# jonaselgammal/GPry

Hardware: AMD Instinct MI355X
Metric: gp_refit_plus_nora_acq_cycle_throughput (higher is better)
Workload: dtype f64

## Files before the change

gpry_amd/_lib.py:

```python
import ctypes as C
import ctypes as _ct
import os

import numpy as np

_HERE = os.path.dirname(os.path.abspath(__file__))
LIB_PATH = os.path.join(_HERE, "libgpry_hip.so")

GPRY_MAX_DIM = 32
MASK_CLASSIFIED_INF = 1
MASK_OUTSIDE_TRUST = 2

KERNEL_IDS = {"rbf": 0, "matern12": 1, "matern32": 2, "matern52": 3}
KERNEL_WHITE = 0x10


class GpryAffine(C.Structure):
    _fields_ = [("has_x_affine", C.c_int),
                ("x_lo", C.c_double * GPRY_MAX_DIM),
                ("x_span", C.c_double * GPRY_MAX_DIM),
                ("y_mean", C.c_double), ("y_std", C.c_double),
                ("clip_hi", C.c_double)]


# ... 40 lines not shown
    "gpry_ns_generation_clustered": (C.c_int, [_vp, _vp, _vp, _vp, _vp, C.c_int64, C.c_double, _vp, C.c_uint64,
                                               C.c_int64, C.c_int, C.c_int, _vp, C.c_int, _vp, _vp, _vp,
                                               _P(C.c_double)]),
    "gpry_ns_generation_volumes": (C.c_int, [_vp, _vp, _vp, _vp, _vp, C.c_int64, C.c_double, _vp, C.c_uint64,
                                             C.c_int64, C.c_int, C.c_int, _vp, C.c_int, _vp, _vp, _vp, _vp,
                                             _P(C.c_double)]),
    "gpry_ns_generation_phantoms": (C.c_int, [_vp, _vp, _vp, _vp, _vp, C.c_int64, C.c_double, _vp, C.c_uint64,
                                              C.c_int64, C.c_int, C.c_int, _vp, C.c_int, _vp, _vp, _vp, _vp, C.c_int,
                                              _vp, _vp, _P(C.c_double)]),
    "gpry_ns_knn": (C.c_int, [_vp, _vp, _vp, _vp, C.c_int64, C.c_int, _vp, _P(C.c_double)]),
    "gpry_mcmc_chains": (C.c_int, [_vp, _vp, _vp, _vp, _vp, C.c_int64, _vp, C.c_double, C.c_double, C.c_uint64,
                                   C.c_int64, C.c_int, C.c_int, _vp, _vp, _vp, _vp, _vp, _vp, _vp, _vp, _P(C.c_double)]),
    "gpry_mcmc_ladders": (C.c_int, [_vp, _vp, _vp, _vp, _vp, C.c_int64, C.c_int, _vp, _vp, C.c_double, C.c_uint64,
                                    C.c_int64, C.c_int, C.c_int, C.c_int] + [_vp] * 11 + [_P(C.c_double)]),
    "gpry_hmc_chains": (C.c_int, [_vp, _vp, _vp, _vp, _vp, C.c_int64, _vp, C.c_double, C.c_int, C.c_double, C.c_double,
                                  C.c_uint64, C.c_int64, C.c_int, C.c_int] + [_vp] * 12),
    "gpry_hmc_chains_reflect": (C.c_int, [_vp, _vp, _vp, _vp, _vp, C.c_int64, _vp, C.c_double, C.c_int, C.c_double,
                                          C.c_double, C.c_uint64, C.c_int64, C.c_int, C.c_int] + [_vp] * 11
                                + [C.c_int, C.c_int, _vp, _vp]),
    "gpry_maximize_mean": (C.c_int, [_vp, _vp, _vp, _vp, _vp, C.c_int64, _vp, _vp, C.c_int, C.c_int, C.c_double,
                                     C.c_double, C.c_double] + [_vp] * 12 + [_P(C.c_double)]),
    "gpry_maximize_acq": (C.c_int, [_vp, _vp, _vp, _vp, C.c_int64, _vp, _vp, C.c_double, C.c_double, C.c_double, C.c_int,
                                    C.c_int, C.c_double, C.c_double, C.c_double] + [_vp] * 14 + [_P(C.c_double)]),
    "gpry_hessian_mean": (C.c_int, [_vp, _vp, C.c_int64, _vp, _vp, _vp, _P(C.c_double)]),
    "gpry_mean_theta_grad": (C.c_int, [_vp, _vp, C.c_int64, _vp, _vp, _P(C.c_double)]),
    "gpry_predict_thetas": (C.c_int, [_vp, _vp, C.c_int64, _vp, C.c_int64, _vp, _vp, _vp, _P(C.c_double)]),
    "gpry_predict_thetas_var": (C.c_int, [_vp, _vp, C.c_int64, _vp, C.c_int64, _vp, _vp, _vp, _vp, _P(C.c_double)]),
    "gpry_predict_cov": (C.c_int, [_vp, _vp, C.c_int64, _vp, _vp, _vp, _P(C.c_double)]),
    "gpry_sample_joint": (C.c_int, [_vp, _vp, C.c_int64, _vp, C.c_int64, C.c_uint64, C.c_double, _vp, _vp, _vp, _vp,
                                    _P(C.c_int), _P(C.c_double), _P(C.c_double)]),
    "gpry_loo": (C.c_int, [_vp, _vp, _vp, _vp, _vp, _vp, _P(C.c_double)]),
    "gpry_svm_fit": (C.c_int, [_vp, _vp, _vp, C.c_int64, C.c_int64, C.c_double, C.c_double, C.c_double, C.c_int64, _vp,
                               _P(C.c_double), _P(C.c_double), _P(C.c_double), _P(C.c_int64), _P(C.c_int), _P(C.c_double)]),
    "gpry_leave_out": (C.c_int, [_vp, _vp, _vp, C.c_int64, _vp, _vp, _vp, _vp, _vp, _P(C.c_double)]),
    "gpry_predict_without": (C.c_int, [_vp, _vp, _vp, C.c_int64, _vp, C.c_int64, _vp, _vp, _vp, _P(C.c_double)]),
    "gpry_var_theta_grad": (C.c_int, [_vp, _vp, C.c_int64, _vp, _vp, _P(C.c_double)]),
    "gpry_var_theta_grad_panel": (C.c_int64, [_vp]),
    "gpry_predict_grad": (C.c_int, [_vp, _vp, C.c_int, _vp, _vp, _vp]),
    "gpry_predict_grad_batch": (C.c_int, [_vp, _vp, C.c_int64, C.c_int, _vp, _vp, _vp, _vp]),
    "gpry_predict_point": (C.c_int, [_vp, _vp, C.c_int, C.c_int, _vp, _vp, _vp, _vp, _vp]),
    "gpry_set_gates": (C.c_int, [_vp, _vp, _vp, C.c_int64, C.c_double, C.c_double, C.c_int, _vp]),
    "gpry_sweep_logexp": (C.c_int, [_vp, _vp, C.c_int64, _vp, C.c_double, C.c_double,
                                    C.c_double, _vp, _vp, _vp, _P(C.c_int64)]),
    "gpry_sweep_logexp_given": (C.c_int, [_vp, _vp, C.c_int64, _vp, _vp, _vp, C.c_double, C.c_double,
                                          C.c_double, _vp, _vp, _vp, _P(C.c_int64)]),
    "gpry_sweep_fetch": (C.c_int, [_vp, C.c_int64, _vp, _vp, _vp]),
    "gpry_sweep_prune_info": (C.c_int, [_vp, _vp, _vp]),
    "gpry_sweep_screen_info": (C.c_int, [_vp, _vp]),
    "gpry_sweep_topk": (C.c_int, [_vp, C.c_int64, _vp, C.c_int64, _vp, _P(C.c_int64),
                                  _P(C.c_double)]),
    "gpry_kb_reset": (C.c_int, [_vp]),
    "gpry_kb_register": (C.c_int, [_vp, _vp, C.c_int64, _P(C.c_int64), _vp]),
    "gpry_kb_gram": (C.c_int, [_vp, C.c_int64, _vp, _vp, _P(C.c_int64)]),
    "gpry_kb_gram_rows": (C.c_int, [_vp, _vp, C.c_int64, _vp, _vp, _P(C.c_int64)]),
    "gpry_kb_rank": (C.c_int, [_vp, _vp, C.c_int64, _vp, C.c_int64, _vp, _vp, _vp, _vp, C.c_int64, _vp, C.c_int64, _vp,
                               C.c_int64, _vp, _vp, _vp, _vp, _vp, _P(C.c_int64), _P(C.c_int64), _vp]),
    "gpry_comm_unique_id": (C.c_int, [_vp]),
    "gpry_comm_init": (C.c_int, [_vp, C.c_int, C.c_int, _vp, _P(_vp)]),
    "gpry_comm_destroy": (C.c_int, [_vp]),
    "gpry_comm_info": (C.c_int, [_vp, _P(C.c_int), _P(C.c_int), _P(C.c_int)]),
    "gpry_comm_allgather": (C.c_int, [_vp, _vp, C.c_int64, _vp]),
    "gpry_comm_allreduce_max": (C.c_int, [_vp, _vp, C.c_int64]),
    "gpry_comm_barrier": (C.c_int, [_vp]),
    "gpry_group_create": (C.c_int, [C.c_int, _P(C.c_int), _vp, _P(_vp)]),
    "gpry_group_destroy": (C.c_int, [_vp]),
    "gpry_group_size": (C.c_int, [_vp, _P(C.c_int), _P(C.c_int)]),
    "gpry_group_member": (_vp, [_vp, C.c_int]),
    "gpry_group_last_error": (C.c_char_p, [_vp]),
    "gpry_group_set_model": (C.c_int, [_vp, _vp, _vp, _vp, C.c_int64, C.c_int, C.c_int, _vp,
                                       _P(GpryAffine), _P(C.c_int)]),
    "gpry_group_set_gates": (C.c_int, [_vp, _vp, _vp, C.c_int64, C.c_double, C.c_double, C.c_int, _vp]),
    "gpry_group_sweep_logexp": (C.c_int, [_vp, _vp, C.c_int64, _vp, C.c_double, C.c_double,
                                          C.c_double, _vp, _vp, _vp, _P(C.c_int64)]),
    "gpry_group_sweep_logexp_given": (C.c_int, [_vp, _vp, C.c_int64, _vp, _vp, _vp, C.c_double, C.c_double,
                                                C.c_double, _vp, _vp, _vp, _P(C.c_int64)]),
    "gpry_group_sweep_fetch": (C.c_int, [_vp, C.c_int64, _vp, _vp, _vp]),
    "gpry_group_sweep_topk": (C.c_int, [_vp, C.c_int64, _vp, C.c_int64, _vp, _P(C.c_int64),
                                        _P(C.c_double), _P(C.c_int)]),
    "gpry_group_lml_batch": (C.c_int, [_vp, _vp, C.c_int, C.c_int, _vp, _vp, _vp]),
    "gpry_timing_reset": (C.c_int, [_vp]),
    "gpry_timing_get": (C.c_int, [_vp, C.c_char_p, _P(C.c_double), _P(C.c_int64)]),
    "gpry_sweep_info": (C.c_int, [_vp, _P(C.c_int), _vp]),
    "gpry_microbench": (C.c_int, [_vp, C.c_int, C.c_int64, _P(C.c_double)]),
    "gpry_debug_gemm": (C.c_int, [_vp, _vp, _vp, _vp] + [C.c_int] * 9),
    "gpry_debug_logexp": (C.c_int, [_vp, _vp, _vp, C.c_int64, C.c_double, C.c_double, C.c_double, _vp]),
}


def _given_arrays(y_given, sigma_given, M):
    if y_given is None:
        raise ValueError("sigma_given without y_given")
    y_given = np.ascontiguousarray(y_given, dtype=np.float64)
    if y_given.shape != (M,):
        raise ValueError(f"y_given has shape {y_given.shape}, the pool has {M} rows")
    if sigma_given is not None:
        sigma_given = np.ascontiguousarray(sigma_given, dtype=np.float64)
        if sigma_given.shape != (M,):
            raise ValueError(f"sigma_given has shape {sigma_given.shape}, the pool has {M} rows")
    return y_given, sigma_given


MAX_STATUS = ("CONVERGED_G", "CONVERGED_F", "STALLED", "MAXITER", "BAD_START", "BAD_GRADIENT")


class GpryHipError(RuntimeError):
    """An API / HIP / RCCL failure reported by libgpry_hip.so."""


_lib = None


def load_library(path=None):
    global _lib
    if _lib is not None and path is None:
        return _lib
    p = path or os.environ.get("GPRY_HIP_LIB", LIB_PATH)
    if not os.path.exists(p):
        raise GpryHipError(
            f"{p} not found. Build it with `python -c 'import __graft_entry__ as g; "
            "g.build()'` or `make -C gpry_amd/csrc`. There is no CPU fallback.")
    lib = C.CDLL(p)
    for name, (res, args) in SIGNATURES.items():
        fn = getattr(lib, name)
        fn.restype, fn.argtypes = res, args
    _lib = lib
    return lib


def _ptr(a):
    return None if a is None else a.ctypes.data_as(C.c_void_p)


def _ptrs(arrays, *keys):
    return [_ptr(arrays.get(k)) for k in keys]


_CHAIN_OUT = ("X", "y", "X_last", "y_last", "naccept", "ncalls")
_BFGS_OUT = ("iters", "ncalls", "ngrad", "status")
_BFGS_TR = ("G_tr", "nhalv_tr", "reset_tr")


def _f64(a, shape=None):
    a = np.ascontiguousarray(a, dtype=np.float64)
    if shape is not None and a.shape != shape:
        raise ValueError(f"expected shape {shape}, got {a.shape}")
    return a


def device_count():
    n = C.c_int(0)
    lib = load_library()
    if lib.gpry_device_count(C.byref(n)) != 0:
        return 0
    return n.value


def make_affine(x_lo=None, x_span=None, y_mean=0.0, y_std=1.0, clip_hi=np.inf):
    tf = GpryAffine()
    tf.has_x_affine = 0 if x_lo is None else 1
    if x_lo is not None:
        for k in range(len(x_lo)):
            tf.x_lo[k] = float(x_lo[k])
            tf.x_span[k] = float(x_span[k])
    tf.y_mean, tf.y_std = float(y_mean), float(y_std)
    tf.clip_hi = float(clip_hi)
    return tf
# ... 689 lines not shown
    def sweep_topk(self, Kp, exclude=None):
        Kp = int(Kp)
        top = np.zeros(max(Kp, 1), dtype=CAND_DTYPE)
        n_out, bound = C.c_int64(0), C.c_double(0.0)
        if exclude is not None and len(exclude):
            exclude = np.ascontiguousarray(np.sort(np.asarray(exclude, dtype=np.int64)))
            nex = len(exclude)
        else:
            exclude, nex = None, 0
        self._check(self._lib.gpry_sweep_topk(self._h, Kp, _ptr(exclude), nex, _ptr(top),
                                              C.byref(n_out), C.byref(bound)), "gpry_sweep_topk")
        return top[:n_out.value], bound.value

    def kb_reset(self):
        self._check(self._lib.gpry_kb_reset(self._h), "gpry_kb_reset")

    def kb_register(self, X, want_var0=True):
        X = _f64(X)
        m = X.shape[0]
        first = C.c_int64(0)
        var0 = np.empty(m) if want_var0 else None
        self._check(self._lib.gpry_kb_register(self._h, _ptr(X), m, C.byref(first), _ptr(var0)),
                    "gpry_kb_register")
        return first.value, var0

    def kb_gram(self, p, n):
        G, kv = np.empty(n), np.empty(n)
        nn = C.c_int64(0)
        self._check(self._lib.gpry_kb_gram(self._h, int(p), _ptr(G), _ptr(kv), C.byref(nn)),
                    "gpry_kb_gram")
        if nn.value != n:
            raise GpryHipError(f"kb_gram: device holds {nn.value} candidates, host expected {n}")
        return G, kv

    def kb_gram_rows(self, p, n):
        p = np.ascontiguousarray(p, dtype=np.int64)
        G, kv = np.empty((len(p), n)), np.empty((len(p), n))
        nn = C.c_int64(0)
        self._check(self._lib.gpry_kb_gram_rows(self._h, _ptr(p), len(p), _ptr(G), _ptr(kv), C.byref(nn)),
                    "gpry_kb_gram_rows")
        if nn.value != n:
            raise GpryHipError(f"kb_gram_rows: device holds {nn.value} candidates, host expected {n}")
        return G, kv

    def kb_rank(self, X_new, var0, idx, y, sigma, acq, order, params, slots):
        m_new = 0 if X_new is None else len(X_new)
        X_new = None if m_new == 0 else _f64(X_new)
        params = _f64(params)
        counter, info = C.c_int64(0), C.c_int64(0)
        stats = np.zeros(3, dtype=np.int64)
        s_idx, s_y, s_sigma, s_acq, s_cond = slots
        for a, t in ((var0, np.float64), (idx, np.int64), (y, np.float64), (sigma, np.float64), (acq, np.float64),
                     (order, np.int64), (s_idx, np.int64), (s_y, np.float64), (s_sigma, np.float64),
                     (s_acq, np.float64), (s_cond, np.float64)):
            if a.dtype != t or not a.flags.c_contiguous:
                raise ValueError("kb_rank: arrays must be contiguous int64 / float64")
        if not (len(y) == len(sigma) == len(acq) == len(idx)) or len(params) != 5 or \
                not (len(s_idx) == len(s_y) == len(s_sigma) == len(s_acq) == len(s_cond)):
            raise ValueError("kb_rank: array lengths do not match")
        self._check(self._lib.gpry_kb_rank(self._h, _ptr(X_new), m_new, _ptr(var0), len(var0), _ptr(idx), _ptr(y),
                                           _ptr(sigma), _ptr(acq), len(idx), _ptr(order), len(order), _ptr(params),
                                           len(s_idx) - 1, _ptr(s_idx), _ptr(s_y), _ptr(s_sigma), _ptr(s_acq),
                                           _ptr(s_cond), C.byref(counter), C.byref(info), _ptr(stats)), "gpry_kb_rank")
        return counter.value, info.value, stats

    def timing_reset(self):
        self._check(self._lib.gpry_timing_reset(self._h), "gpry_timing_reset")

    def timing(self, name):
        ms, cnt = C.c_double(0.0), C.c_int64(0)
        self._lib.gpry_timing_get(self._h, name.encode(), C.byref(ms), C.byref(cnt))
        return ms.value, cnt.value

    def debug_gemm(self, A, B, C0, M, N, K, a_trans=False, b_trans=False, epi=0, kmode=0,
                   lower_only=False, tile_map=0):
        A, B = _f64(A), _f64(B)
        crow = (M + 127) // 128 if epi == 3 else M
        Cout = np.ascontiguousarray(np.zeros((crow, N)) if C0 is None else C0, dtype=np.float64).copy()
        self._check(self._lib.gpry_debug_gemm(self._h, _ptr(A), _ptr(B), _ptr(Cout), M, N, K,
                                              int(a_trans), int(b_trans), int(epi), int(kmode),
                                              int(lower_only), int(tile_map)), "gpry_debug_gemm")
        return Cout

    def debug_logexp(self, mu, sigma, zeta, baseline, sigma_n):
        mu, sigma = _f64(mu), _f64(sigma)
        acq = np.empty(len(mu))
        self._check(self._lib.gpry_debug_logexp(self._h, _ptr(mu), _ptr(sigma), len(mu), float(zeta),
                                                float(baseline), float(sigma_n), _ptr(acq)), "gpry_debug_logexp")
        return acq


    def microbench(self, kind, nbytes=0):
        v = C.c_double(0.0)
        self._check(self._lib.gpry_microbench(self._h, int(kind), int(nbytes), C.byref(v)),
                    "gpry_microbench")
        return v.value


class DeviceGroup:

    def __init__(self, devices, adopt=None):
        self._lib = load_library()
        devices = [int(v) for v in devices]
        if not devices:
            raise ValueError("DeviceGroup needs at least one device")
        self.devices = devices
        self._adopt = adopt
        arr = (C.c_int * len(devices))(*devices)
        self._h = C.c_void_p()
        rc = self._lib.gpry_group_create(len(devices), arr, adopt._h if adopt is not None else None,
                                         C.byref(self._h))
        if rc != 0:
            msg = self._lib.gpry_group_last_error(None).decode(errors="replace")
            self._h = None
            raise GpryHipError(f"gpry_group_create({devices}) failed ({rc}): {msg}")
        n, tr = C.c_int(0), C.c_int(0)
        self._lib.gpry_group_size(self._h, C.byref(n), C.byref(tr))
        self.size, self.transport = n.value, {0: "host", 1: "rccl"}[tr.value]
        self.note = self._lib.gpry_group_last_error(self._h).decode(errors="replace")
        self.sweep_epoch = 0
        self._sweep_M = 0
        self.d = 0

    def _check(self, rc, what):
        if rc != 0:
            msg = self._lib.gpry_group_last_error(self._h).decode(errors="replace")
            raise GpryHipError(f"{what} failed ({rc}): {msg}")

    def close(self):
        if getattr(self, "_h", None):
            try:
                self._lib.gpry_group_destroy(self._h)
            except Exception:
                pass
            self._h = None

    def __del__(self):
        self.close()

    def member(self, i):
        h = self._lib.gpry_group_member(self._h, int(i))
        if not h:
            raise IndexError(i)
        v = Device._view(h, self.devices[i])
        v._group = self
        return v

    def set_model(self, X_, y_, alpha, kernel_id, theta, affine=None):
        X_ = _f64(X_)
        N, d = X_.shape
        y_ = _f64(y_, (N,))
        alpha = _f64(np.broadcast_to(alpha, (N,)))
        if int(kernel_id) & KERNEL_WHITE:
            raise NotImplementedError("a device group does not carry the white term (WhiteKernel) of the kernel yet")
        theta = _f64(theta, (d + 1,))
        tf = make_affine(*affine) if affine is not None else None
        info = C.c_int(0)
        self._check(self._lib.gpry_group_set_model(self._h, _ptr(X_), _ptr(y_), _ptr(alpha), N, d, int(kernel_id),
                                                   _ptr(theta), C.byref(tf) if tf is not None else None,
                                                   C.byref(info)), "gpry_group_set_model")
        self.d = d
        return info.value

    def set_gates(self, sv=None, coef=None, gamma=0.0, intercept=0.0, positive_is_finite=True,
                  trust_bounds=None):
        n_sv = 0
# ... 113 lines not shown
```

gpry_amd/csrc/api.hip:

```cpp
#include "sweep.h"
#include "kb_gram.h"
#include <algorithm>

int require_model(gpry_ctx* ctx, bool need_factor) {
    if (ctx->N <= 0) return gpry_fail(ctx, -1, "no training set (call gpry_set_train)");
    if (!ctx->have_theta) return gpry_fail(ctx, -1, "no hyperparameters (call gpry_set_theta)");
    if (need_factor && !ctx->factor_valid) return gpry_fail(ctx, -1, "model not factorised (call gpry_factorize)");
    if (need_factor && ctx->tf.has_x_affine)
        for (int k = 0; k < ctx->d; k++)
            if (!(ctx->tf.x_span[k] != 0.0) || !isfinite(ctx->tf.x_span[k]) || !isfinite(ctx->tf.x_lo[k]))
                return gpry_fail(ctx, -1, "affine map of X: span %g, offset %g in dimension %d of %d (gpry_set_affine of another model?)",
                                 ctx->tf.x_span[k], ctx->tf.x_lo[k], k, ctx->d);
    return 0;
}


static int copy_out_matrix(gpry_ctx* ctx, const double* dsrc, int64_t ld, int64_t rows, int64_t cols, double* hdst) {
    HIP_TRY(ctx, hipMemcpy2DAsync(hdst, sizeof(double) * cols, dsrc, sizeof(double) * ld,
                                  sizeof(double) * cols, rows, hipMemcpyDeviceToHost, ctx->stream));
    HIP_TRY(ctx, hipStreamSynchronize(ctx->stream));
    return 0;
}

bool panel_timed_out(int marker) { return (marker & 0xFF00) == 0x5A00; }
int panel_timeout_error(gpry_ctx* ctx, int marker) {
    return gpry_fail(ctx, -2, "Cholesky panel step timed out (wait %d; the GPU is shared with work that starves the step?)", marker & 0xFF);
}

int objective_entry(gpry_ctx* ctx, const char* name, const double* thetas, int64_t B) {
    GPRY_TRY(serve_stop(ctx));
    if (ctx->N <= 0) return gpry_fail(ctx, -1, "%s: no training set (call gpry_set_train)", name);
    const int w = ctx_ntheta(ctx);
    for (int64_t i = 0; i < B * w; i++)
        if (!isfinite(thetas[i]))
            return gpry_fail(ctx, -1, "%s: theta[%d] of evaluation %lld is not finite", name, (int)(i % w), (long long)(i / w));
    if (ctx->d > 32) return gpry_fail(ctx, -1, "%s: d > 32 is not supported", name);
    HIP_TRY(ctx, hipSetDevice(ctx->device));
    ctx->lml_cache = false;
    return 0;
}
int objective_row(gpry_ctx* ctx, int64_t bytes, int info_at, double** hres, double** dres) {
    GPRY_TRY(ensure_pinned(ctx, bytes));
    *hres = static_cast<double*>(ctx->hpin);
    *dres = static_cast<double*>(ctx->hpin_dev);
    objective_row_unwritten(*hres, info_at);
    return 0;
}
int objective_status(gpry_ctx* ctx, const char* name, int64_t which, const double* row, int info_at, int* info) {
    if (row[info_at] < 0.0) return gpry_fail(ctx, -2, "%s: evaluation %lld did not deliver its status", name, (long long)which);
    if (panel_timed_out((int)row[info_at + 2])) return panel_timeout_error(ctx, (int)row[info_at + 2]);
    const int i0 = (int)row[info_at], i1 = (int)row[info_at + 1];
    *info = i0 != 0 ? i0 : i1;
    return 0;
}
int objective_wait(gpry_ctx* ctx, const char* name, int rc, const double* row, int info_at, int* info) {
    const hipError_t e = hipStreamSynchronize(ctx->stream);
    if (rc) return rc;
    if (e != hipSuccess) return gpry_fail(ctx, -2, "%s: %s", name, hipGetErrorString(e));
    return row ? objective_status(ctx, name, 0, row, info_at, info) : 0;
}
void objective_write(const gpry_ctx* ctx, int info, double head, const double* g, const double* h, double* value, double* grad,
                     double* hess) {
    const int w = ctx_ntheta(ctx);
    const bool pd = info == 0;
    *value = pd ? head - 0.5 * (double)ctx->N * log(2.0 * M_PI) : -INFINITY;
    if (grad) for (int k = 0; k < w; k++) grad[k] = pd ? g[k] : 0.0;
    if (hess) for (int k = 0; k < w * w; k++) hess[k] = pd ? h[k] : 0.0;
}

int build_factor(gpry_ctx* ctx, double* A, double* V, double* T, int* info_host) {
    GPRY_TRY(launch_scale_train(ctx));
    const bool want_stacked = ctx->opt_chol != 1 && potrf_stacked_usable(ctx, ctx->Np);
    {
        StageScope s(ctx, "kernel_build");
        GPRY_TRY(launch_kernel_train(ctx, A, 1, want_stacked ? T : nullptr));
    }
    if (ctx->opt_chol == 1) {
        StageScope s(ctx, "potrf");
        GPRY_TRY(rocsolver_potrf_trtri(ctx, A, V, ctx->Np, 1));
    } else {
        bool piped = false;
        struct PipeGuard {
            gpry_ctx* c; bool armed = false;
            ~PipeGuard() { if (armed) trtri_pipeline_abort(c); }
        } guard{ctx};
        if (ctx->opt_factor_pipeline && ctx->opt_chol == 0 && ctx->Np >= ctx->opt_factor_pipeline_min && ctx->bn == 1 && !ctx->tp &&
            !potrf_stacked_usable(ctx, ctx->Np)) {
            const int rc = trtri_pipeline_begin(ctx, A, V, T, ctx->Np);
            if (rc < 0) return rc;
            piped = rc == 0;
            guard.armed = piped;
        }
        bool stacked = !piped && want_stacked;
        if (stacked) {
            StageScope s(ctx, "potrf");
            const int rc = potrf_stacked(ctx, A, T, ctx->Np);
            if (rc < 0) return rc;
            stacked = rc == 0;
        }
        if (stacked) {
            StageScope s(ctx, "trtri");
            GPRY_TRY(transpose_upper_launch(ctx, T, V, ctx->Np));
        } else {
            {
                StageScope s(ctx, "potrf");
                GPRY_TRY(ctx->opt_chol_overlap ? potrf_lower_overlap(ctx, A, ctx->Np) : potrf_lower_fused(ctx, A, ctx->Np));
            }
            {
                StageScope s(ctx, "trtri");
                if (piped) { GPRY_TRY(trtri_pipeline_finish(ctx)); guard.armed = false; }
                else GPRY_TRY(trtri_lower(ctx, A, V, T, ctx->Np));
            }
        }
    }
    ctx->info_cleared = false;
    if (!info_host) return 0;
    int info[4] = {0, 0, 0, 0};
    HIP_TRY(ctx, hipMemcpyAsync(info, ctx->dinfo, 4 * sizeof(int), hipMemcpyDeviceToHost, ctx->stream));
    HIP_TRY(ctx, hipStreamSynchronize(ctx->stream));
    if (panel_timed_out(info[3])) return panel_timeout_error(ctx, info[3]);
    *info_host = info[0] != 0 ? info[0] : info[1];
    return 0;
}

constexpr int RES_INFO = LML_RES_INFO;
static_assert(RES_INFO + 3 <= GPRY_BRES_STRIDE, "result row too short");
int lml_chain(gpry_ctx* ctx, int want_grad, double* dres) {
    GPRY_TRY(build_factor(ctx, ctx->dW, ctx->dW2, ctx->dW3, nullptr));
    double* dz = ctx->dvec;
    double* da = ctx->dvec + ctx->Np;
    double* dout = ctx->dvec + 2 * ctx->Np;
    {
        StageScope s(ctx, "solve_alpha");
        GPRY_TRY(solve_alpha(ctx, ctx->dW2, ctx->dy, dz, da, ctx->Np));
        GPRY_TRY(logdet_and_quad(ctx, ctx->dW, dz, ctx->Np, dout, want_grad ? nullptr : dres, RES_INFO));
    }
    if (!want_grad) return 0;
    {
        StageScope s(ctx, "lauum");
        GPRY_TRY(lauum_lower(ctx, ctx->dW2, ctx->dW3, ctx->Np));
    }
    StageScope s(ctx, "lml_traces");
    return launch_lml_traces(ctx, ctx->dW3, da, dout + 2, dout, dres, RES_INFO);
}

struct BatchLayout {
    int64_t w, w2, w3, xs, vec, part, split, par, info;
    int64_t part_cap, split_cap, stride;
};
static int batch_layout(gpry_ctx* ctx, const BatchChain& bc, BatchLayout* L) {
    const int64_t Np = ctx->Np, nn = Np * Np;
    int slices = 0;
    GPRY_TRY(factor_chain_slices(ctx, Np, &slices));
    const int DPsel = dp_class(ctx->d);
    const int64_t nb = Np / 64, ntile = nb * (nb + 1) / 2;
    const int64_t p1 = ((Np + 255) / 256) * Np, p2 = ntile * (DPsel + 2);
    int64_t o = 0;
    auto take = [&](int64_t n) { const int64_t at = o; o += round_up(n, 32); return at; };
    L->w = take(nn); L->w2 = take(nn); L->w3 = take(nn);
    L->xs = take(Np * ctx->dpad);
    L->vec = take(8 * Np + 4096);
    L->part_cap = p1 > p2 ? p1 : p2;
    if (L->part_cap < bc.part_min) L->part_cap = bc.part_min;
    L->part = take(L->part_cap);
    L->split_cap = (int64_t)slices * nn;
    if (L->split_cap < bc.split_min) L->split_cap = bc.split_min;
    L->split = take(L->split_cap > 0 ? L->split_cap : 1);
    L->par = take(GPRY_BPAR_ROW);
    L->info = take(8);
    L->stride = o + 32 * 9;
    return 0;
}
static int ensure_batch_buffers(gpry_ctx* ctx, int64_t arena_doubles, int64_t res_bytes) {
    if (arena_doubles > ctx->barena_cap) {
        if (ctx->barena) GPRY_TRY(dev_free(ctx, ctx->barena));
        ctx->barena = nullptr; ctx->barena_cap = 0;
        const hipError_t e = hipMalloc((void**)&ctx->barena, sizeof(double) * (size_t)arena_doubles);
        if (e == hipErrorOutOfMemory) { (void)hipGetLastError(); ctx->barena = nullptr; return 2; }
        if (e != hipSuccess) { ctx->barena = nullptr; return gpry_fail(ctx, -2, "batched objective: hipMalloc of the scratch arena failed: %s", hipGetErrorString(e)); }
        ctx->barena_cap = arena_doubles;
    }
    if (res_bytes > ctx->hbres_cap) {
        if (ctx->hbres) HIP_TRY(ctx, hipHostFree(ctx->hbres));
        ctx->hbres = nullptr; ctx->hbres_dev = nullptr; ctx->hbres_cap = 0;
        HIP_TRY(ctx, hipHostMalloc(&ctx->hbres, (size_t)res_bytes, hipHostMallocMapped | hipHostMallocPortable));
        HIP_TRY(ctx, hipHostGetDevicePointer(&ctx->hbres_dev, ctx->hbres, 0));
        memset(ctx->hbres, 0, (size_t)res_bytes);
        ctx->hbres_cap = res_bytes;
    }
    return 0;
}
static bool lml_batch_usable(const gpry_ctx* ctx) {
    return ctx->N > 0 && ctx->Np > 128 && ctx->Np <= ctx->opt_lml_batch && ctx->d <= 32 && ctx->opt_chol == 0;
}
static const BatchChain LML_BATCH = {"lml_batch", lml_chain, false, 0, 0, 2, RES_INFO, lml_head};
int objective_batch_general(gpry_ctx* ctx, const BatchChain& bc, const double* thetas, int64_t B, int want_grad, double* lml, double* grad,
                            int* info) {
    const int w = ctx_ntheta(ctx);
    struct Scope {
        gpry_ctx* c;
        double *dW, *dW2, *dW3, *dXs, *dvec, *dpart, *dsplit; int* dinfo; hipStream_t stream;
        int64_t part_cap, split_cap; bool xs_foreign, have_theta;
        double theta[GPRY_THETA_MAX];
        explicit Scope(gpry_ctx* ctx) : c(ctx), dW(ctx->dW), dW2(ctx->dW2), dW3(ctx->dW3), dXs(ctx->dXs), dvec(ctx->dvec), dpart(ctx->dpart),
                                        dsplit(ctx->dsplit), dinfo(ctx->dinfo), stream(ctx->stream), part_cap(ctx->part_cap), split_cap(ctx->split_cap),
                                        xs_foreign(ctx->xs_foreign), have_theta(ctx->have_theta) {
            memcpy(theta, ctx->theta, sizeof(theta));
        }
        ~Scope() {
            c->dW = dW; c->dW2 = dW2; c->dW3 = dW3; c->dXs = dXs; c->dvec = dvec; c->dpart = dpart; c->dsplit = dsplit; c->dinfo = dinfo;
            c->stream = stream;
            c->part_cap = part_cap; c->split_cap = split_cap; c->xs_foreign = xs_foreign; c->have_theta = have_theta;
            c->info_cleared = false;
            memcpy(c->theta, theta, sizeof(theta));
            c->bn = 1; c->bstride = 0; c->bpar = nullptr; c->tp = false;
        }
    } scope(ctx);
    const bool tp = !bc.latency_only && ctx->opt_lml_schedule == 1;
    ctx->tp = tp;
    BatchLayout L;
    GPRY_TRY(batch_layout(ctx, bc, &L));
    int64_t chunk = B < 96 ? B : 96;
    int64_t mem_cap = (ctx->opt_lml_batch_mb << 20) / (8 * L.stride);
// ... 718 lines not shown
        GPRY_TRY(dev_alloc(ctx, &nX, cap * ctx->dpad));
        GPRY_TRY(dev_alloc(ctx, &nO, 2 * cap));
        if (ctx->kb_n > 0) {
            HIP_TRY(ctx, hipMemcpyAsync(nU, ctx->dU, sizeof(double) * ctx->kb_n * Np, hipMemcpyDeviceToDevice, st));
            HIP_TRY(ctx, hipMemcpyAsync(nX, ctx->dXkb, sizeof(double) * ctx->kb_n * ctx->dpad, hipMemcpyDeviceToDevice, st));
        }
        HIP_TRY(ctx, hipStreamSynchronize(st));
        if (ctx->dU) GPRY_TRY(dev_free(ctx, ctx->dU));
        if (ctx->dXkb) GPRY_TRY(dev_free(ctx, ctx->dXkb));
        if (ctx->dkbout) GPRY_TRY(dev_free(ctx, ctx->dkbout));
        ctx->dU = nU; ctx->dXkb = nX; ctx->dkbout = nO; ctx->kb_cap = cap; ctx->kb_ld = Np;
    }
    const int64_t mp = round_up(m, 128);
    TmpBuf<double> bX, bpar;
    GPRY_TRY(bX.alloc(ctx, m * ctx->d));
    GPRY_TRY(bpar.alloc(ctx, 3 * GPRY_MAX_DIM));
    double *dX = bX.p, *dpar = bpar.p;
    HIP_TRY(ctx, hipMemcpyAsync(dX, X, sizeof(double) * m * ctx->d, hipMemcpyHostToDevice, st));
    double hpar[3 * GPRY_MAX_DIM];
    for (int k = 0; k < GPRY_MAX_DIM; k++) {
        hpar[k] = k < ctx->d ? ctx->tf.x_lo[k] : 0.0;
        hpar[GPRY_MAX_DIM + k] = k < ctx->d ? ctx->tf.x_span[k] : 1.0;
        hpar[2 * GPRY_MAX_DIM + k] = k < ctx->d ? exp(ctx->theta[1 + k]) : 1.0;
    }
    HIP_TRY(ctx, hipMemcpyAsync(dpar, hpar, sizeof(hpar), hipMemcpyHostToDevice, st));
    hipLaunchKernelGGL(scale_rows_kernel, dim3((unsigned)((m * ctx->dpad + 255) / 256)), dim3(256), 0, st, dX, m,
                       ctx->d, ctx->dpad, ctx->tf.has_x_affine, dpar, dpar + GPRY_MAX_DIM, dpar + 2 * GPRY_MAX_DIM,
                       ctx->dXkb + ctx->kb_n * ctx->dpad);
    GPRY_TRY(dev_grow(ctx, &ctx->dKst, &ctx->kst_cap, Np * mp));
    int64_t saveM = ctx->sw_M; ctx->sw_M = m;
    int rc = mp <= 512 ? launch_cross_build_small(ctx, dX, 0, mp, mp, ctx->dKst, nullptr, 1)
                       : launch_cross_build(ctx, dX, 0, mp, mp, ctx->dKst, nullptr, 1);
    ctx->sw_M = saveM;
    if (rc) return rc;
    GemmArgs g = {};
    g.A = ctx->dKst; g.lda = mp;
    g.B = ctx->dV; g.ldb = Np;
    g.C = ctx->dU + ctx->kb_n * Np; g.ldc = Np;
    g.M = (int)mp; g.N = (int)Np; g.K = (int)Np;
    g.kmode = KM_B_UPPER; g.lower_only = 0; g.tile_map = TM_ROWMAJOR;
    {
        int ns = 1;
        while (ns < 8 && Np / (ns * 2) >= 256) ns *= 2;
        if (ns > 1) {
            GPRY_TRY(gemm_split_scratch(ctx, ns, mp * Np, &g.split_buf));
            g.nsplit = ns; g.split_stride = mp * Np;
        }
    }
    GPRY_TRY(gemm_f64_launch(ctx, g, true, true, EPI_STORE));
    if (var0) {
        hipLaunchKernelGGL(kb_var0_kernel, dim3((unsigned)((m + 3) / 4)), dim3(256), 0, st, ctx->dU, Np, ctx->kb_n, m,
                           Np, ctx_prior_var(ctx), ctx->dkbout);
        HIP_TRY(ctx, hipMemcpyAsync(var0, ctx->dkbout, sizeof(double) * m, hipMemcpyDeviceToHost, st));
    }
    HIP_TRY(ctx, hipStreamSynchronize(st));
    if (first) *first = ctx->kb_n;
    ctx->kb_n += m;
    return 0;
}

int gpry_kb_gram(gpry_ctx* ctx, int64_t p, double* G, double* kvec, int64_t* n) {
    if (!ctx) return gpry_fail(nullptr, -1, "gpry_kb_gram: ctx is NULL");
    GPRY_TRY(require_model(ctx, true));
    HIP_TRY(ctx, hipSetDevice(ctx->device));
    if (p < 0 || p >= ctx->kb_n) return gpry_fail(ctx, -1, "kb_gram: index %lld out of range [0, %lld)", (long long)p, (long long)ctx->kb_n);
    StageScope kb_scope(ctx, "kb_gram");
    hipStream_t st = ctx->stream;
    int64_t nn = ctx->kb_n;
    GPRY_TRY(ensure_pinned(ctx, (int64_t)sizeof(double) * 2 * nn));
    double* hres = static_cast<double*>(ctx->hpin);
    double* dres = static_cast<double*>(ctx->hpin_dev);
    hipLaunchKernelGGL(kb_gram_kernel, dim3((unsigned)((nn + 3) / 4)), dim3(256), 0, st, ctx->dU, ctx->Np, nn, p,
                       ctx->Np, ctx->dXkb, ctx->dpad, ctx->kernel_id, exp(ctx->theta[0]), dres, dres + nn);
    HIP_TRY(ctx, hipGetLastError());
    HIP_TRY(ctx, hipStreamSynchronize(st));
    memcpy(G, hres, sizeof(double) * nn);
    memcpy(kvec, hres + nn, sizeof(double) * nn);
    if (n) *n = nn;
    return 0;
}

}

extern "C" int gpry_debug_gemm(gpry_ctx* ctx, const double* A, const double* B, double* C, int M, int N,
                               int K, int a_trans, int b_trans, int epi, int kmode, int lower_only,
                               int tile_map) {
    if (!ctx) return gpry_fail(nullptr, -1, "gpry_debug_gemm: ctx is NULL");
    GPRY_TRY(serve_stop(ctx));
    if (!A || !B || !C) return gpry_fail(ctx, -1, "debug_gemm: A, B and C must not be NULL");
    HIP_TRY(ctx, hipSetDevice(ctx->device));
    if (M % 64 || N % 64 || K % 64) return gpry_fail(ctx, -1, "debug_gemm: dims must be multiples of 64");
    int64_t crow = (epi == EPI_SUMSQ) ? (M + 127) / 128 : M;
    TmpBuf<double> bA, bB, bC;
    GPRY_TRY(bA.alloc(ctx, (int64_t)M * K));
    GPRY_TRY(bB.alloc(ctx, (int64_t)K * N));
    GPRY_TRY(bC.alloc(ctx, crow * N));
    double *dA = bA.p, *dB = bB.p, *dC = bC.p;
    hipStream_t st = ctx->stream;
    HIP_TRY(ctx, hipMemcpyAsync(dA, A, sizeof(double) * M * K, hipMemcpyHostToDevice, st));
    HIP_TRY(ctx, hipMemcpyAsync(dB, B, sizeof(double) * K * N, hipMemcpyHostToDevice, st));
    HIP_TRY(ctx, hipMemcpyAsync(dC, C, sizeof(double) * crow * N, hipMemcpyHostToDevice, st));
    GemmArgs g = {};
    g.A = dA; g.lda = a_trans ? M : K;
    g.B = dB; g.ldb = b_trans ? K : N;
    g.C = dC; g.ldc = N;
    g.M = M; g.N = N; g.K = K; g.kmode = kmode; g.lower_only = lower_only; g.tile_map = tile_map & 0xff;
    g.small64 = (tile_map >> 28) & 1;
    const int nsplit = (tile_map >> 8) & 15;
    if (nsplit > 1) {
        GPRY_TRY(gemm_split_scratch(ctx, nsplit, (int64_t)crow * N, &g.split_buf));
        g.nsplit = nsplit; g.split_stride = (int64_t)crow * N;
    }
    const int seg = (tile_map >> 16) & 0xfff;
    if (seg > 0) {
        if (M % 128 || N % 128 || K % 32) return gpry_fail(ctx, -1, "debug_gemm: stream-K needs M, N multiples of 128, K of 32");
        GemmPartsPlan pl;
        std::vector<GemmShape> sh = {{M, N, K}};
        GPRY_TRY(gemm_parts_plan_build(ctx, kmode, lower_only, sh, seg, &pl));
        int rc = gemm_dma_parts_launch(ctx, g, a_trans != 0, b_trans != 0, epi, pl, (int64_t)crow * N);
        if (rc == 0 && hipStreamSynchronize(st) != hipSuccess) rc = gpry_fail(ctx, -2, "debug_gemm: stream-K launch failed");
        gemm_parts_plan_free(&pl);
        if (rc) return rc;
    } else {
        StageScope s(ctx, "debug_gemm");
        GPRY_TRY(gemm_f64_launch(ctx, g, a_trans != 0, b_trans != 0, epi));
    }
    HIP_TRY(ctx, hipMemcpyAsync(C, dC, sizeof(double) * crow * N, hipMemcpyDeviceToHost, st));
    HIP_TRY(ctx, hipStreamSynchronize(st));
    return 0;
}

extern "C" int gpry_debug_logexp(gpry_ctx* ctx, const double* mu, const double* sigma, int64_t n, double zeta,
                                 double baseline, double sigma_n, double* acq) {
    if (!ctx) return gpry_fail(nullptr, -1, "gpry_debug_logexp: ctx is NULL");
    if (n <= 0) return 0;
    if (!mu || !sigma || !acq) return gpry_fail(ctx, -1, "debug_logexp: mu, sigma and acq must not be NULL");
    HIP_TRY(ctx, hipSetDevice(ctx->device));
    TmpBuf<double> bd;
    GPRY_TRY(bd.alloc(ctx, 3 * n));
    double* d = bd.p;
    hipStream_t st = ctx->stream;
    HIP_TRY(ctx, hipMemcpyAsync(d, mu, sizeof(double) * n, hipMemcpyHostToDevice, st));
    HIP_TRY(ctx, hipMemcpyAsync(d + n, sigma, sizeof(double) * n, hipMemcpyHostToDevice, st));
    GPRY_TRY(launch_logexp(ctx, d, d + n, n, zeta, baseline, sigma_n, d + 2 * n));
    HIP_TRY(ctx, hipMemcpyAsync(acq, d + 2 * n, sizeof(double) * n, hipMemcpyDeviceToHost, st));
    HIP_TRY(ctx, hipStreamSynchronize(st));
    return 0;
}
```

gpry_amd/csrc/chol.hip:

```cpp
#include "common.h"
#include <algorithm>
#include <dlfcn.h>

__global__ __launch_bounds__(64) void trtri_diag_kernel(const double* __restrict__ L_,
                                                        double* __restrict__ V_, int64_t ld,
                                                        const int* info, int64_t bstride) {
    __shared__ double Lk[64 * 64];
    if (*bset(info, (int)blockIdx.z, bstride) != 0) return;
    const double* __restrict__ L = bset(L_, (int)blockIdx.z, bstride);
    double* __restrict__ V = bset(V_, (int)blockIdx.z, bstride);
    const int t = threadIdx.x;
    const int64_t b0 = (int64_t)blockIdx.x * 64;
    for (int e = t; e < 64 * 64; e += 64) {
        int i = e >> 6, j = e & 63;
        Lk[e] = L[(b0 + i) * ld + b0 + j];
    }
    __syncthreads();
    double x[64];
#pragma unroll
    for (int i = 0; i < 64; i++) {
        double s = (i == t) ? 1.0 : 0.0;
#pragma unroll
        for (int k = 0; k < i; k++) s = fma(-Lk[i * 64 + k], x[k], s);
        x[i] = (i >= t) ? s / Lk[i * 64 + i] : 0.0;
    }
#pragma unroll
    for (int i = 0; i < 64; i++) V[(b0 + i) * ld + b0 + t] = x[i];
}

struct TriNode { int lo, mid, hi, level; };
static int build_tree(int lo, int hi, std::vector<TriNode>& out) {
    if (hi - lo <= 1) return 0;
    int mid = lo + (hi - lo + 1) / 2;
    int l1 = build_tree(lo, mid, out), l2 = build_tree(mid, hi, out);
    int lev = (l1 > l2 ? l1 : l2) + 1;
    out.push_back({lo, mid, hi, lev});
    return lev;
}

struct TrtriPhaseLevel {
    int lev = 0;
    int64_t t_first = 0, v_first = 0;
    int n_t = 0, n_v = 0, mM_t = 0, mN_t = 0, mM_v = 0, mN_v = 0;
    GemmPartsPlan sk_t, sk_v;
};
struct TrtriPhase {
    int blocks_done = 0, diag_lo = 0, diag_hi = 0;
    std::vector<TrtriPhaseLevel> levels;
};
struct TrtriPlan {
    int64_t Np = 0;
    int leaf = 1;
    std::vector<GemmBatchItem*> d_t, d_v;
    std::vector<int> count, maxM, maxN;
    std::vector<int> aligned;
    std::vector<TrtriPhase> phases;
    GemmBatchItem* d_phase_items = nullptr;
    std::vector<int> seg_t, seg_v;
    std::vector<GemmPartsPlan> sk_t, sk_v;
    GemmPartsPlan sk_lauum;
    int seg_lauum = 0;
    void release() {
        for (auto p : d_t) if (p) (void)hipFree(p);
        for (auto p : d_v) if (p) (void)hipFree(p);
        if (d_phase_items) (void)hipFree(d_phase_items);
        for (auto& q : sk_t) gemm_parts_plan_free(&q);
        for (auto& q : sk_v) gemm_parts_plan_free(&q);
        for (auto& ph : phases) for (auto& pv : ph.levels) { gemm_parts_plan_free(&pv.sk_t); gemm_parts_plan_free(&pv.sk_v); }
        gemm_parts_plan_free(&sk_lauum);
    }
};
void trtri_plan_free(gpry_ctx* ctx) {
    TrtriPlan* pl = static_cast<TrtriPlan*>(ctx->trtri_plan);
    if (!pl) return;
    pl->release();
    delete pl;
    ctx->trtri_plan = nullptr;
}

static int trtri_plan_get(gpry_ctx* ctx, int64_t Np, TrtriPlan** out) {
    if (!ctx->trtri_plan) ctx->trtri_plan = new TrtriPlan();
    TrtriPlan& pl = *static_cast<TrtriPlan*>(ctx->trtri_plan);
    if (pl.Np == Np) { *out = &pl; return 0; }
    pl.release();
    pl = TrtriPlan();
    int slots = 512;
    { hipDeviceProp_t prop; if (hipGetDeviceProperties(&prop, ctx->device) == hipSuccess && prop.multiProcessorCount > 0) slots = 2 * prop.multiProcessorCount; }
    pl.leaf = (Np > 128 && Np <= 1024) ? 2 : 1;
    std::vector<TriNode> nodes;
    int nlev = build_tree(0, (int)(Np / (64 * pl.leaf)), nodes);
    for (auto& nd : nodes) { nd.lo *= pl.leaf; nd.mid *= pl.leaf; nd.hi *= pl.leaf; }
    for (int lev = 1; lev <= nlev; lev++) {
        std::vector<GemmBatchItem> bt, bv;
        int mM = 0, mN = 0, al = 1;
        for (auto& nd : nodes) {
            if (nd.level != lev) continue;
            int64_t lo = nd.lo * 64, mid = nd.mid * 64, hi = nd.hi * 64;
            int m = (int)(hi - mid), n = (int)(mid - lo);
            GemmBatchItem a;
            a.a_off = mid * Np + lo; a.b_off = lo * Np + lo; a.c_off = mid * Np + lo;
            a.M = m; a.N = n; a.K = n; a.pad = 0;
            bt.push_back(a);
            GemmBatchItem b;
            b.a_off = mid * Np + mid; b.b_off = mid * Np + lo; b.c_off = mid * Np + lo;
            b.M = m; b.N = n; b.K = m; b.pad = 0;
            bv.push_back(b);
            if (m > mM) mM = m;
            if (n > mN) mN = n;
            if (m % 128 || n % 128) al = 0;
        }
        GemmBatchItem *dt = nullptr, *dv = nullptr;
        size_t bytes = bt.size() * sizeof(GemmBatchItem);
        hipError_t e = hipMalloc(&dt, bytes);
        if (e == hipSuccess) e = hipMalloc(&dv, bytes);
        if (e == hipSuccess) e = hipMemcpy(dt, bt.data(), bytes, hipMemcpyHostToDevice);
        if (e == hipSuccess) e = hipMemcpy(dv, bv.data(), bytes, hipMemcpyHostToDevice);
        if (e != hipSuccess) {
            if (dt) (void)hipFree(dt);
            if (dv) (void)hipFree(dv);
            pl.release();
            pl = TrtriPlan();
            return gpry_fail(ctx, -2, "trtri plan (Np = %lld): %s", (long long)Np, hipGetErrorString(e));
        }
        pl.d_t.push_back(dt); pl.d_v.push_back(dv);
        pl.count.push_back((int)bt.size()); pl.maxM.push_back(mM); pl.maxN.push_back(mN);
        pl.aligned.push_back(al);
        pl.seg_t.push_back(0); pl.seg_v.push_back(0);
        pl.sk_t.emplace_back(); pl.sk_v.emplace_back();
        if (al && mN >= 512 && Np <= ctx->opt_gemm_streamk) {
            std::vector<GemmShape> st_, sv_;
            for (auto& a : bt) st_.push_back({a.M, a.N, a.K});
            for (auto& b : bv) sv_.push_back({b.M, b.N, b.K});
            pl.seg_t.back() = gemm_parts_segment(KM_B_LOWER, 0, st_, slots);
            pl.seg_v.back() = gemm_parts_segment(KM_A_LOWER, 0, sv_, slots);
            int rc = gemm_parts_plan_build(ctx, KM_B_LOWER, 0, st_, pl.seg_t.back(), &pl.sk_t.back());
            if (rc == 0) rc = gemm_parts_plan_build(ctx, KM_A_LOWER, 0, sv_, pl.seg_v.back(), &pl.sk_v.back());
            if (rc) { pl.release(); pl = TrtriPlan(); return rc; }
        }
    }
    if (Np >= 512 && Np <= ctx->opt_gemm_streamk) {
        std::vector<GemmShape> sh = {{(int)Np, (int)Np, (int)Np}};
        pl.seg_lauum = gemm_parts_segment(KM_AT_LOWER_B_LOWER, 1, sh, slots);
        int rc = gemm_parts_plan_build(ctx, KM_AT_LOWER_B_LOWER, 1, sh, pl.seg_lauum, &pl.sk_lauum);
        if (rc) { pl.release(); pl = TrtriPlan(); return rc; }
    }
    const int nblk = (int)(Np / 64);
    if (nblk >= 8) {
        const TriNode root = nodes.back();
        std::vector<int> cps = {root.mid, nblk};
        for (auto& nd : nodes)
            if (nd.lo == root.lo && nd.hi == root.mid) cps.push_back(nd.mid);
        const int spine = nblk / 2;
        for (int lo = root.mid, hi = root.hi; hi - lo >= spine && hi - lo > 1;) {
            int mid = -1;
            for (auto& nd : nodes) if (nd.lo == lo && nd.hi == hi) mid = nd.mid;
            if (mid < 0) break;
            cps.push_back(mid);
            lo = mid;
        }
        std::sort(cps.begin(), cps.end());
        cps.erase(std::unique(cps.begin(), cps.end()), cps.end());
        auto phase_of = [&](int blocks) { size_t p = 0; while (cps[p] < blocks) p++; return p; };
        std::vector<GemmBatchItem> all;
        int dlo = 0;
        for (size_t p = 0; p < cps.size(); p++) {
            TrtriPhase ph;
            ph.blocks_done = cps[p]; ph.diag_lo = dlo; ph.diag_hi = cps[p]; dlo = cps[p];
            for (int lev = 1; lev <= nlev; lev++) {
                TrtriPhaseLevel pv; pv.lev = lev - 1;
                std::vector<GemmBatchItem> bt, bv;
                for (auto& nd : nodes) {
                    if (nd.level != lev) continue;
                    int64_t lo = nd.lo * 64, mid = nd.mid * 64, hi = nd.hi * 64;
                    int m = (int)(hi - mid), n = (int)(mid - lo);
                    if (phase_of(nd.mid) == p) {
                        GemmBatchItem a;
                        a.a_off = mid * Np + lo; a.b_off = lo * Np + lo; a.c_off = mid * Np + lo;
                        a.M = m; a.N = n; a.K = n; a.pad = 0;
                        bt.push_back(a);
                        if (m > pv.mM_t) pv.mM_t = m;
                        if (n > pv.mN_t) pv.mN_t = n;
                    }
                    if (phase_of(nd.hi) == p) {
                        GemmBatchItem b;
                        b.a_off = mid * Np + mid; b.b_off = mid * Np + lo; b.c_off = mid * Np + lo;
                        b.M = m; b.N = n; b.K = m; b.pad = 0;
                        bv.push_back(b);
                        if (m > pv.mM_v) pv.mM_v = m;
                        if (n > pv.mN_v) pv.mN_v = n;
                    }
                }
                if (bt.empty() && bv.empty()) continue;
                if (pl.seg_t[lev - 1] > 0) {
                    std::vector<GemmShape> st_, sv_;
                    for (auto& a : bt) st_.push_back({a.M, a.N, a.K});
                    for (auto& b : bv) sv_.push_back({b.M, b.N, b.K});
                    int rc = gemm_parts_plan_build(ctx, KM_B_LOWER, 0, st_, pl.seg_t[lev - 1], &pv.sk_t);
                    if (rc == 0) rc = gemm_parts_plan_build(ctx, KM_A_LOWER, 0, sv_, pl.seg_v[lev - 1], &pv.sk_v);
                    if (rc) { ph.levels.push_back(pv); pl.phases.push_back(ph); pl.release(); pl = TrtriPlan(); return rc; }
                }
                pv.n_t = (int)bt.size(); pv.n_v = (int)bv.size();
                pv.t_first = (int64_t)all.size(); all.insert(all.end(), bt.begin(), bt.end());
                pv.v_first = (int64_t)all.size(); all.insert(all.end(), bv.begin(), bv.end());
                ph.levels.push_back(pv);
            }
            pl.phases.push_back(ph);
        }
        hipError_t e = hipMalloc(&pl.d_phase_items, all.size() * sizeof(GemmBatchItem));
        if (e == hipSuccess) e = hipMemcpy(pl.d_phase_items, all.data(), all.size() * sizeof(GemmBatchItem), hipMemcpyHostToDevice);
        if (e != hipSuccess) {
            pl.release();
            pl = TrtriPlan();
            return gpry_fail(ctx, -2, "trtri plan (Np = %lld): %s", (long long)Np, hipGetErrorString(e));
        }
    }
    pl.Np = Np;
    *out = &pl;
    return 0;
}

static int trtri_level_nsplit(gpry_ctx* ctx, const TrtriPlan* pl, size_t lev) {
    if (ctx->tp) return 1;
    const int tm = (pl->maxM[lev] + 127) / 128, tn = (pl->maxN[lev] + 127) / 128;
    const int64_t tiles = (int64_t)tm * tn * pl->count[lev];
    int nsplit = 1;
    if (pl->maxN[lev] >= 512) {
        while (nsplit < 4 && tiles * nsplit * 2 <= 1024 && pl->maxN[lev] / (nsplit * 2) >= 128) nsplit *= 2;
    }
    return nsplit;
}

static int trtri_level_products(gpry_ctx* ctx, const double* L, double* V, double* T, int64_t Np, int nsplit, int aligned,
                                const GemmBatchItem* d_t, int n_t, int mM_t, int mN_t,
                                const GemmBatchItem* d_v, int n_v, int mM_v, int mN_v, hipStream_t st,
                                const GemmPartsPlan* sk_t = nullptr, const GemmPartsPlan* sk_v = nullptr) {
    if (sk_t && sk_v && Np <= ctx->opt_gemm_streamk && !ctx->tp) {
        if (n_t > 0) {
            GemmArgs g = {};
            g.A = L; g.lda = Np; g.B = V; g.ldb = Np; g.C = T; g.ldc = Np;
            g.kmode = KM_B_LOWER; g.batch = d_t; g.n_batch = n_t; g.info = ctx->dinfo; g.stream = st;
            GPRY_TRY(gemm_dma_parts_launch(ctx, g, false, false, EPI_STORE, *sk_t, Np * Np));
        }
        if (n_v > 0) {
            GemmArgs h = {};
            h.A = V; h.lda = Np; h.B = T; h.ldb = Np; h.C = V; h.ldc = Np;
            h.kmode = KM_A_LOWER; h.batch = d_v; h.n_batch = n_v; h.info = ctx->dinfo; h.stream = st;
            GPRY_TRY(gemm_dma_parts_launch(ctx, h, false, false, EPI_STORE_NEG, *sk_v, Np * Np));
        }
        return 0;
    }
    double* sbuf = nullptr;
    if (nsplit > 1) GPRY_TRY(gemm_split_scratch(ctx, nsplit, Np * Np, &sbuf));
    if (n_t > 0) {
        GemmArgs g = {};
        g.A = L; g.lda = Np; g.B = V; g.ldb = Np; g.C = T; g.ldc = Np;
        g.M = mM_t; g.N = mN_t; g.K = 0;
        g.kmode = KM_B_LOWER; g.lower_only = 0; g.tile_map = TM_ROWMAJOR;
        g.batch = d_t; g.n_batch = n_t; g.info = ctx->dinfo; g.stream = st;
        g.nsplit = nsplit; g.split_buf = sbuf; g.split_stride = Np * Np; g.dma_ok = aligned;
        g.small64 = 1;
        GPRY_TRY(gemm_f64_launch(ctx, g, false, false, EPI_STORE));
    }
    if (n_v > 0) {
        GemmArgs h = {};
        h.A = V; h.lda = Np; h.B = T; h.ldb = Np; h.C = V; h.ldc = Np;
        h.M = mM_v; h.N = mN_v; h.K = 0;
        h.kmode = KM_A_LOWER; h.lower_only = 0; h.tile_map = TM_ROWMAJOR;
        h.batch = d_v; h.n_batch = n_v; h.info = ctx->dinfo; h.stream = st;
        h.nsplit = nsplit; h.split_buf = sbuf; h.split_stride = Np * Np; h.dma_ok = aligned;
        h.small64 = 1;
        GPRY_TRY(gemm_f64_launch(ctx, h, false, false, EPI_STORE_NEG));
    }
    return 0;
}

__global__ __launch_bounds__(256) void zero_sets_kernel(double2* __restrict__ p_, int64_t n2, int64_t bstride) {
    double2* __restrict__ p = bset(p_, (int)blockIdx.z, bstride);
    const int64_t stride = (int64_t)gridDim.x * blockDim.x;
    for (int64_t i = (int64_t)blockIdx.x * blockDim.x + threadIdx.x; i < n2; i += stride) p[i] = make_double2(0.0, 0.0);
}

int trtri_lower(gpry_ctx* ctx, const double* L, double* V, double* T, int64_t Np) {
    hipStream_t st = ctx->stream;
    const bool single_wave = Np <= 128;
    const bool clear_in_diag = !single_wave && Np <= 1024;
    const bool tp_min_clear = ctx->tp && !single_wave;
    if (tp_min_clear) {
    } else if (!clear_in_diag && ctx->bn > 1) {
        const int64_t n2 = Np * Np / 2;
        int64_t nb = (n2 + 2047) / 2048;
        if (nb > 4096) nb = 4096;
        hipLaunchKernelGGL(zero_sets_kernel, dim3((unsigned)nb, 1, (unsigned)ctx->bn), dim3(256), 0, st, reinterpret_cast<double2*>(V), n2,
                           ctx->bstride);
        HIP_TRY(ctx, hipGetLastError());
    } else if (!clear_in_diag) HIP_TRY(ctx, hipMemsetAsync(V, 0, sizeof(double) * Np * Np, st));
    TrtriPlan* pl = nullptr;
    GPRY_TRY(trtri_plan_get(ctx, Np, &pl));
    if (single_wave) {
        hipLaunchKernelGGL(trtri_diag_kernel, dim3((unsigned)(Np / 64), 1, (unsigned)ctx->bn), dim3(64), 0, st, L, V, Np, ctx->dinfo,
                           ctx->bstride);
        HIP_TRY(ctx, hipGetLastError());
    } else if (pl->leaf == 2) {
        GPRY_TRY(launch_trtri_diag128(ctx, L, V, Np, st, !tp_min_clear));
    } else {
        GPRY_TRY(launch_trtri_diag(ctx, L, V, Np, st, tp_min_clear));
    }
    for (size_t lev = 0; lev < pl->count.size(); lev++)
        GPRY_TRY(trtri_level_products(ctx, L, V, T, Np, trtri_level_nsplit(ctx, pl, lev), pl->aligned[lev],
                                      pl->d_t[lev], pl->count[lev], pl->maxM[lev], pl->maxN[lev],
                                      pl->d_v[lev], pl->count[lev], pl->maxM[lev], pl->maxN[lev], st,
                                      pl->seg_t[lev] > 0 ? &pl->sk_t[lev] : nullptr, pl->seg_t[lev] > 0 ? &pl->sk_v[lev] : nullptr));
    return 0;
}

struct TrtriPipe {
    const double* L = nullptr; double* V = nullptr; double* T = nullptr;
    int64_t Np = 0; TrtriPlan* pl = nullptr; size_t next = 0; bool active = false;
    hipStream_t side = nullptr;
};
static TrtriPipe* pipe_of(gpry_ctx* ctx) {
    if (!ctx->trtri_pipe) ctx->trtri_pipe = new TrtriPipe();
    return static_cast<TrtriPipe*>(ctx->trtri_pipe);
}
void trtri_pipe_free(gpry_ctx* ctx) {
    delete static_cast<TrtriPipe*>(ctx->trtri_pipe);
    ctx->trtri_pipe = nullptr;
}
static int trtri_phase_run(gpry_ctx* ctx, TrtriPipe* pp, size_t p, hipStream_t st) {
    const TrtriPlan* pl = pp->pl;
    const TrtriPhase& ph = pl->phases[p];
    if (ph.diag_hi > ph.diag_lo)
        GPRY_TRY(launch_trtri_diag_range(ctx, pp->L, pp->V, pp->Np, ph.diag_lo, ph.diag_hi - ph.diag_lo, st));
    for (const TrtriPhaseLevel& pv : ph.levels)
        GPRY_TRY(trtri_level_products(ctx, pp->L, pp->V, pp->T, pp->Np, trtri_level_nsplit(ctx, pl, (size_t)pv.lev),
                                      pl->aligned[pv.lev], pl->d_phase_items + pv.t_first, pv.n_t, pv.mM_t, pv.mN_t,
                                      pl->d_phase_items + pv.v_first, pv.n_v, pv.mM_v, pv.mN_v, st,
                                      pl->seg_t[pv.lev] > 0 ? &pv.sk_t : nullptr, pl->seg_t[pv.lev] > 0 ? &pv.sk_v : nullptr));
    return 0;
}
int trtri_pipeline_begin(gpry_ctx* ctx, const double* L, double* V, double* T, int64_t Np) {
    TrtriPipe* pp = pipe_of(ctx);
    pp->active = false;
    if (!ctx->stream2) return 1;
    TrtriPlan* pl = nullptr;
    GPRY_TRY(trtri_plan_get(ctx, Np, &pl));
    if (pl->phases.size() < 2 || pl->leaf != 1) return 1;
    while (ctx->ev_pool.size() < pl->phases.size() + 2) {
        hipEvent_t ev;
        HIP_TRY(ctx, hipEventCreateWithFlags(&ev, hipEventDisableTiming));
        ctx->ev_pool.push_back(ev);
    }
    int maxsplit = 1;
    for (size_t lev = 0; lev < pl->count.size(); lev++) {
        const int ns = trtri_level_nsplit(ctx, pl, lev);
        if (ns > maxsplit) maxsplit = ns;
    }
    if (Np <= ctx->opt_gemm_streamk) {
        for (auto& q : pl->sk_t) if (q.max_slices > maxsplit) maxsplit = q.max_slices;
        for (auto& q : pl->sk_v) if (q.max_slices > maxsplit) maxsplit = q.max_slices;
        for (auto& ph : pl->phases) for (auto& pv : ph.levels) {
            if (pv.sk_t.max_slices > maxsplit) maxsplit = pv.sk_t.max_slices;
            if (pv.sk_v.max_slices > maxsplit) maxsplit = pv.sk_v.max_slices;
        }
    }
    double* sbuf = nullptr;
    if (maxsplit > 1) GPRY_TRY(gemm_split_scratch(ctx, maxsplit, Np * Np, &sbuf));
    pp->L = L; pp->V = V; pp->T = T; pp->Np = Np; pp->pl = pl; pp->next = 0; pp->active = true;
    pp->side = ctx->stream2;
    hipEvent_t ev0 = ctx->ev_pool[pl->phases.size()];
    HIP_TRY(ctx, hipEventRecord(ev0, ctx->stream));
    HIP_TRY(ctx, hipStreamWaitEvent(pp->side, ev0, 0));
    HIP_TRY(ctx, hipMemsetAsync(V, 0, sizeof(double) * Np * Np, pp->side));
    return 0;
}
int trtri_pipeline_step(gpry_ctx* ctx, int blocks_done) {
    TrtriPipe* pp = static_cast<TrtriPipe*>(ctx->trtri_pipe);
    if (!pp || !pp->active) return 0;
    const TrtriPlan* pl = pp->pl;
    if (pp->next + 1 >= pl->phases.size() || pl->phases[pp->next].blocks_done != blocks_done) return 0;
    hipEvent_t ev = ctx->ev_pool[pp->next];
    HIP_TRY(ctx, hipEventRecord(ev, ctx->stream));
    HIP_TRY(ctx, hipStreamWaitEvent(pp->side, ev, 0));
    GPRY_TRY(trtri_phase_run(ctx, pp, pp->next, pp->side));
    pp->next++;
    return 0;
}
int trtri_pipeline_finish(gpry_ctx* ctx) {
    TrtriPipe* pp = static_cast<TrtriPipe*>(ctx->trtri_pipe);
    if (!pp || !pp->active) return gpry_fail(ctx, -1, "trtri_pipeline_finish without begin");
    pp->active = false;
    const TrtriPlan* pl = pp->pl;
    hipEvent_t evd = ctx->ev_pool[pl->phases.size() + 1];
    HIP_TRY(ctx, hipEventRecord(evd, pp->side));
    HIP_TRY(ctx, hipStreamWaitEvent(ctx->stream, evd, 0));
    for (; pp->next < pl->phases.size(); pp->next++) GPRY_TRY(trtri_phase_run(ctx, pp, pp->next, ctx->stream));
    return 0;
}

void trtri_pipeline_abort(gpry_ctx* ctx) {
    TrtriPipe* pp = static_cast<TrtriPipe*>(ctx->trtri_pipe);
    if (!pp || !pp->active) return;
    pp->active = false;
    if (pp->side) (void)hipStreamSynchronize(pp->side);
}

int lauum_lower(gpry_ctx* ctx, const double* V, double* Kinv, int64_t Np) {
    if (Np >= 512 && Np <= ctx->opt_gemm_streamk && !ctx->tp) {
        TrtriPlan* pl = nullptr;
        GPRY_TRY(trtri_plan_get(ctx, Np, &pl));
        GemmArgs g = {};
        g.A = V; g.lda = Np; g.B = V; g.ldb = Np; g.C = Kinv; g.ldc = Np;
        g.M = (int)Np; g.N = (int)Np; g.K = (int)Np;
        g.kmode = KM_AT_LOWER_B_LOWER; g.lower_only = 1; g.info = ctx->dinfo;
        return gemm_dma_parts_launch(ctx, g, true, false, EPI_STORE, pl->sk_lauum, Np * Np);
    }
    GemmArgs g = {};
    g.A = V; g.lda = Np; g.B = V; g.ldb = Np; g.C = Kinv; g.ldc = Np;
    g.M = (int)Np; g.N = (int)Np; g.K = (int)Np;
    g.kmode = KM_AT_LOWER_B_LOWER; g.lower_only = 1; g.tile_map = TM_ROWMAJOR; g.info = ctx->dinfo;
    const int64_t tiles = (Np / 128) * (Np / 128 + 1) / 2;
    const int nsplit = ctx->tp ? 1 : splitk_count(tiles, Np);
    if (nsplit > 1) {
        double* sbuf = nullptr;
        GPRY_TRY(gemm_split_scratch(ctx, nsplit, Np * Np, &sbuf));
        g.nsplit = nsplit; g.split_buf = sbuf; g.split_stride = Np * Np;
    }
    g.small64 = 1;
    return gemm_f64_launch(ctx, g, true, false, EPI_STORE);
}

int factor_chain_slices(gpry_ctx* ctx, int64_t Np, int* slices) {
    if (ctx->tp) { *slices = 0; return 0; }
    TrtriPlan* pl = nullptr;
    GPRY_TRY(trtri_plan_get(ctx, Np, &pl));
    int m = 1;
    for (size_t lev = 0; lev < pl->count.size(); lev++) {
        if (pl->seg_t[lev] > 0 && Np <= ctx->opt_gemm_streamk) {
            if (pl->sk_t[lev].max_slices > m) m = pl->sk_t[lev].max_slices;
            if (pl->sk_v[lev].max_slices > m) m = pl->sk_v[lev].max_slices;
        } else {
            const int ns = trtri_level_nsplit(ctx, pl, lev);
            if (ns > m) m = ns;
        }
    }
    if (Np >= 512 && Np <= ctx->opt_gemm_streamk) {
        if (pl->sk_lauum.max_slices > m) m = pl->sk_lauum.max_slices;
    } else {
        const int nsplit = splitk_count((Np / 128) * (Np / 128 + 1) / 2, Np);
        if (nsplit > m) m = nsplit;
    }
    *slices = m > 1 ? m : 0;
    return 0;
}

__global__ __launch_bounds__(256) void trmv_lower_kernel(const double* __restrict__ V_, int64_t ld,
                                                         const double* __restrict__ y,
                                                         double* __restrict__ z_, int64_t n, int64_t bstride) {
    const double* __restrict__ V = bset(V_, (int)blockIdx.z, bstride);
    double* __restrict__ z = bset(z_, (int)blockIdx.z, bstride);
    const int lane = threadIdx.x & 63;
    const int64_t row = (int64_t)blockIdx.x * 4 + (threadIdx.x >> 6);
    if (row >= n) return;
    double s = 0.0;
    for (int64_t k0 = lane; k0 <= row; k0 += 512) {
        double v[8], yy[8];
#pragma unroll
        for (int u = 0; u < 8; u++) {
            const int64_t k = k0 + 64 * u;
            const bool in = k <= row;
            v[u] = in ? V[row * ld + k] : 0.0;
            yy[u] = in ? y[k] : 0.0;
        }
#pragma unroll
        for (int u = 0; u < 8; u++) s = fma(v[u], yy[u], s);
    }
#pragma unroll
    for (int off = 32; off >= 1; off >>= 1) s += __shfl_xor(s, off);
    if (lane == 0) z[row] = s;
}
__global__ __launch_bounds__(256) void trmv_lower_t_kernel(const double* __restrict__ V_, int64_t ld,
                                                           const double* __restrict__ z_,
                                                           double* __restrict__ part_, int64_t n, int64_t bstride) {
    __shared__ double red[4][64];
    const double* __restrict__ V = bset(V_, (int)blockIdx.z, bstride);
    const double* __restrict__ z = bset(z_, (int)blockIdx.z, bstride);
    double* __restrict__ part = bset(part_, (int)blockIdx.z, bstride);
    const int c = threadIdx.x & 63, rq = threadIdx.x >> 6;
    const int64_t col = (int64_t)blockIdx.x * 64 + c;
    const int64_t r0 = (int64_t)blockIdx.y * 256;
    double s = 0.0;
    if (r0 + 255 >= (int64_t)blockIdx.x * 64) {
        for (int q0 = 0; q0 < 64; q0 += 8) {
            double v[8], zz[8];
#pragma unroll
            for (int u = 0; u < 8; u++) {
                const int64_t r = r0 + rq + 4 * (q0 + u);
                const bool in = r >= col && r < n;
                v[u] = in ? V[r * ld + col] : 0.0;
                zz[u] = in ? z[r] : 0.0;
            }
#pragma unroll
            for (int u = 0; u < 8; u++) s = fma(v[u], zz[u], s);
        }
    }
    red[rq][c] = s;
    __syncthreads();
    if (rq == 0) part[(int64_t)blockIdx.y * n + col] = (red[0][c] + red[1][c]) + (red[2][c] + red[3][c]);
}
__global__ void colsum_kernel(const double* __restrict__ part_, int64_t n, int nchunk, double* __restrict__ out_, int64_t bstride) {
    const double* __restrict__ part = bset(part_, (int)blockIdx.z, bstride);
    double* __restrict__ out = bset(out_, (int)blockIdx.z, bstride);
    int64_t col = (int64_t)blockIdx.x * blockDim.x + threadIdx.x;
    if (col >= n) return;
    double s = 0.0;
    for (int ch = 0; ch < nchunk; ch++) s += part[(int64_t)ch * n + col];
    out[col] = s;
}

int solve_alpha(gpry_ctx* ctx, const double* V, const double* y, double* z, double* alpha, int64_t Np) {
    hipStream_t st = ctx->stream;
    const unsigned bn = (unsigned)ctx->bn;
    hipLaunchKernelGGL(trmv_lower_kernel, dim3((unsigned)((Np + 3) / 4), 1, bn), dim3(256), 0, st, V, Np, y, z, Np, ctx->bstride);
    int nchunk = (int)((Np + 255) / 256);
    int64_t need = (int64_t)nchunk * Np;
    if (need > ctx->part_cap && ctx->bpar) return gpry_fail(ctx, -1, "batched chain: partial sums exceed the arena");
    if (need > ctx->part_cap) {
        if (ctx->dpart) dev_free(ctx, ctx->dpart);
        GPRY_TRY(dev_alloc(ctx, &ctx->dpart, need));
// ... 97 lines not shown
```

gpry_amd/csrc/common.h:

```cpp
#pragma once
#include <hip/hip_runtime.h>
#include <stdint.h>
#include <stdio.h>
#include <string.h>
#include <math.h>
#include <string>
#include <vector>
#include <map>

#include "../../include/gpry_hip.h"

#define GPRY_THETA_MAX (2 + GPRY_MAX_DIM)
#define GPRY_BPAR_ROW (2 + GPRY_MAX_DIM)
#define GPRY_BPAR_WHITE (1 + GPRY_MAX_DIM)
#define GPRY_TILE 128
#define GPRY_NB 64

typedef double v4d __attribute__((ext_vector_type(4)));

struct StageTimer {
    double total_ms = 0.0;
    int64_t count = 0;
    std::vector<std::pair<hipEvent_t, hipEvent_t>> pending;
};

struct FinishParams {
    double C, y_mean, y_std, clip_hi, zeta, baseline, sigma_n;
    int want_std, want_acq;
};

struct gpry_ctx {
    int device = 0;
    hipStream_t stream = nullptr;
    hipStream_t stream2 = nullptr;
    std::vector<hipEvent_t> ev_pool;
    char err[1024] = {0};

    int opt_chol = 0;
    int64_t opt_sweep_chunk = 0;
    int opt_timing = 0;
    bool xs_foreign = false;
    bool info_cleared = false;
    int opt_gemm_small = 32;
    int64_t opt_predict_small = 2048;
    int opt_chol_overlap = 1;

    int64_t N = 0, Np = 0, cap = 0;
    int d = 0, dpad = 0, dp_cap = 0;
    int kernel_id = GPRY_RBF;
    bool white = false;
    bool have_theta = false, factor_valid = false;
    double theta[GPRY_THETA_MAX] = {0};
    gpry_affine tf;
    bool lml_cache = false;
    int lml_kernel_id = -1;
    double lml_theta[GPRY_THETA_MAX] = {0};
    int opt_lml_cache = 1;
    unsigned long long lml_seq = 0;
    int opt_lml_small = 1;

    int bn = 1;
    int64_t bstride = 0;
    const double* bpar = nullptr;
    double* barena = nullptr; int64_t barena_cap = 0;
    void* hbres = nullptr; void* hbres_dev = nullptr; int64_t hbres_cap = 0;
    int64_t opt_lml_batch = 4096;
    int64_t opt_lml_batch_mb = 49152;
    int opt_lml_schedule = 0;
    int opt_lml_streams = 2;
    int64_t opt_tp_block = 512;
    int opt_tp_left = 0;
    int64_t opt_tp_tail = 1024;
    int64_t batch_set_doubles = 0, batch_chunk = 0;
    int64_t batch_shrinks = 0;
    int opt_chol_tp_segments = 0;
    int opt_panel_debug = 0;
    bool tp = false;
    std::vector<hipStream_t> tp_streams;
    std::vector<hipEvent_t> tp_events;

    double* dX = nullptr;
    double* dXs = nullptr;
    double* dy = nullptr;
    double* dnoise = nullptr;
    double* dA = nullptr;
    double* dV = nullptr;
    double* dW = nullptr;
    double* dW2 = nullptr;
    double* dW3 = nullptr;
    double* dalpha_ = nullptr;
    double* dvec = nullptr;
    int* dinfo = nullptr;
    double* dparams = nullptr;

    double* gate_sv = nullptr; double* gate_coef = nullptr; double* gate_trust = nullptr;
    int64_t gate_nsv = 0, gate_sv_cap = 0;
    double gate_gamma = 0.0, gate_intercept = 0.0;
    int gate_positive_finite = 1, gate_has_trust = 0, gates_on = 0;

    int64_t sw_M = 0, sw_cap = 0;
    double* dXc = nullptr;
    uint8_t* dmask = nullptr;
    double *dy_all = nullptr, *dsig_all = nullptr, *dacq_all = nullptr;
    struct CandSet {
        int64_t M = 0, cap = 0;
        double* dXc = nullptr; uint8_t* dmask = nullptr;
        double *dy = nullptr, *dsig = nullptr, *dacq = nullptr;
    } pr;
    double* dXcs = nullptr;
    int64_t xcs_cap = 0;
    double* dYcs = nullptr;
    int64_t ycs_cap = 0;
    double xcenter[GPRY_MAX_DIM] = {0};
    double xsum[GPRY_MAX_DIM] = {0};
    double xlo[GPRY_MAX_DIM] = {0}, xhi[GPRY_MAX_DIM] = {0};
    int opt_cross_mfma = 1;
    double alpha_l2 = -1.0;
    double alpha_l1 = 0.0;
    double noise_min = 0.0;
    int panel_form = 0;
    int opt_cross_hybrid = 1;
    double panel_est[4] = {0, 0, 0, 2.5e-7};
    double* dKst = nullptr;
    int64_t kst_cap = 0;
    double* dG = nullptr;
    int64_t g_cap = 0;
    double* dsplit = nullptr;
    int64_t split_cap = 0;
    int opt_predict_split = 1;
    int opt_gemm_dma = 1;
    double* dpart = nullptr;
    int64_t part_cap = 0;
    unsigned long long* dkeys = nullptr; int64_t keys_cap = 0;
    unsigned int* dhist = nullptr;
    unsigned int* dselp = nullptr;
    enum { SELP_HIST_WORDS = 12 * 256, SELP_WORDS = 12 * 256 + 12 * 8 };
    int opt_select_fused = 1;
    int opt_prune_one_select = 1;
    int opt_sweep_small_map = 1;
    gpry_cand* dcand = nullptr; int64_t cand_cap = 0;
    unsigned long long* dsel = nullptr;
    enum { DSEL_NAN = 0,
           DSEL_STATE = 0,
           DSEL_EMIT = 4,
           DSEL_SURV = 6,
           DSEL_GIDX = 7,
           DSEL_LIVE = 8,
           DSEL_FALL = 9,
           DSEL_WORDS = 64 };

    int64_t kb_n = 0, kb_cap = 0;
    int64_t kb_ld = 0;
    double* dU = nullptr;
    double* dXkb = nullptr;
    double* dkbout = nullptr;

    double* dbord = nullptr;
    int64_t bord_cap = 0;
    int64_t n_border = 0;

    void* trtri_plan = nullptr;
    void* trtri_pipe = nullptr;
    int64_t opt_gemm_streamk = 5632;
    int64_t opt_topk_host = 16384;
    int opt_factor_pipeline = 1;
    int opt_factor_pipeline_min = 1280;
    void* chol_plan = nullptr;

    void* srv = nullptr;
    int opt_predict_serve = 1;
    int64_t opt_serve_idle_us = 2000;
    int opt_mcmc_mapped = 0;
    int64_t opt_chol_stacked = 2048;
    int opt_chol_stacked_dense = 0;
    int opt_sweep_overlap = 0;
    int opt_sweep_upload = 1;
    const double* up_X = nullptr;
    const double* up_y = nullptr;
    int up_gates = 0;
    int opt_kb_rank = 1;
    int opt_predict_gates = 0;
    int opt_sweep_prune = 0;
    int opt_sweep_mean_bound = 1;
    int opt_sweep_screen = 1;
    int sw_pruned = 0;
    struct PruneState {
        int have_mask = 0;
        int form = 0;
        FinishParams fp = {};
        int64_t n_eval = 0;
        int64_t rounds = 0, evaluated_total = 0, completed = 0, last_K = 0;
        int64_t n_gidx = 0;
        int tau_done = 0;
        double tau = 0.0;
        int64_t survivors = -1;
        int ybound = 0;
        int64_t live_blocks = 0, blocks = 0;
        int64_t cert_blocks = 0;
    } prune;
    struct ModelSnap {
        double *dV = nullptr, *dalpha_ = nullptr, *dXs = nullptr, *dX = nullptr;
        int64_t v_cap = 0, a_cap = 0, xs_cap = 0, x_cap = 0;
        int64_t N = 0, Np = 0;
        int d = 0, dpad = 0, kernel_id = 0;
        bool white = false;
        double theta[GPRY_THETA_MAX] = {0};
        gpry_affine tf;
        double xcenter[GPRY_MAX_DIM] = {0};
        bool xs_foreign = false;
    } snap;
    double* dub = nullptr;
    int64_t ub_cap = 0;
    double* dXg = nullptr;
    int64_t xg_cap = 0;
    int64_t* dgidx = nullptr;
    int64_t gidx_cap = 0;
    uint8_t* dmc = nullptr;
    int64_t mc_cap = 0;
    uint8_t* dknn = nullptr;
    int64_t knn_cap = 0;
    uint8_t* dph = nullptr;
    int64_t ph_cap = 0;
    uint8_t* djoint = nullptr;
    int64_t joint_cap = 0;
    uint8_t* dloo = nullptr;
    int64_t loo_cap = 0;
    void* hloo = nullptr; int64_t hloo_cap = 0;
    double* dhess = nullptr;
    int64_t hess_cap = 0;
    double* dtg = nullptr;
    int64_t tg_cap = 0;
    uint8_t* dpw = nullptr;
    int64_t pw_cap = 0, pw_np = 0;
    double* dvtg = nullptr;
    int64_t vtg_cap = 0;
    uint8_t* dsvm = nullptr;
    int64_t svm_cap = 0;
    void* hsvm = nullptr; int64_t hsvm_cap = 0;
    int64_t opt_svm_iters = 4096;

    void* hpin = nullptr; void* hpin_dev = nullptr; int64_t hpin_cap = 0;

    std::map<std::string, StageTimer> timers;
};

extern thread_local char g_last_error[1024];

static inline double ctx_white(const gpry_ctx* ctx) { return ctx->white ? exp(ctx->theta[1 + ctx->d]) : 0.0; }
static inline int ctx_ntheta(const gpry_ctx* ctx) { return ctx->d + 1 + (ctx->white ? 1 : 0); }
static inline double ctx_prior_var(const gpry_ctx* ctx) {
    const double C = exp(ctx->theta[0]);
    return ctx->white ? C + exp(ctx->theta[1 + ctx->d]) : C;
}

int gpry_fail(gpry_ctx* ctx, int code, const char* fmt, ...);
static inline int refuse_white(gpry_ctx* ctx, const char* who) {
    if (!ctx->white) return 0;
    return gpry_fail(ctx, -1, "%s: a model with a white term (WhiteKernel, GPRY_KERNEL_WHITE) is not supported by this entry point", who);
}

#define HIP_TRY(ctx, expr)                                                          \
    do {                                                                            \
        hipError_t _e = (expr);                                                     \
        if (_e != hipSuccess)                                                       \
            return gpry_fail(ctx, -2, "%s failed: %s (%s:%d)", #expr,               \
                             hipGetErrorString(_e), __FILE__, __LINE__);            \
    } while (0)

#define GPRY_TRY(expr)                 \
    do {                               \
        int _r = (expr);               \
        if (_r != 0) return _r;        \
    } while (0)

struct StageScope {
    gpry_ctx* ctx; const char* name; hipEvent_t e0 = nullptr, e1 = nullptr; hipStream_t st = nullptr; bool marked = false;
    StageScope(gpry_ctx* c, const char* n, hipStream_t stream = nullptr);
    ~StageScope();
};
void timers_collect(gpry_ctx* ctx);

template <typename T>
int dev_alloc(gpry_ctx* ctx, T** p, int64_t count);
int dev_free(gpry_ctx* ctx, void* p);

static inline int64_t round_up(int64_t a, int64_t b) { return (a + b - 1) / b * b; }
template <typename T>
int dev_grow(gpry_ctx* ctx, T** p, int64_t* cap, int64_t need) {
    if (need <= *cap) return 0;
    HIP_TRY(ctx, hipStreamSynchronize(ctx->stream));
    if (*p) GPRY_TRY(dev_free(ctx, *p));
    *p = nullptr; *cap = 0;
    GPRY_TRY(dev_alloc(ctx, p, need));
    *cap = need;
    return 0;
}

template <typename T>
__device__ __forceinline__ T* bset(T* p, int tb, int64_t bstride) {
    return (T*)((char*)p + (int64_t)tb * bstride * 8);
}
#define GPRY_BRES_STRIDE 40

enum GemmKMode {
    KM_FULL = 0,
    KM_A_LOWER = 1,
    KM_B_LOWER = 2,
    KM_AT_LOWER_B_LOWER = 3,
    KM_B_UPPER = 4,
    KM_AT_LOWER = 5
};
enum GemmEpi { EPI_STORE = 0, EPI_STORE_NEG = 1, EPI_SUB = 2, EPI_SUMSQ = 3 };
enum GemmTileMap { TM_ROWMAJOR = 0, TM_SWEEP = 1, TM_BALANCED = 2 };
#define TM_SWEEP_SMALL (1 << 12)

struct GemmBatchItem { int64_t a_off, b_off, c_off; int M, N, K, pad; };

struct GemmArgs {
    const double* A; const double* B; double* C;
    int64_t lda, ldb, ldc;
    int M, N, K;
    int kmode;
    int lower_only;
    int tile_map;
    const GemmBatchItem* batch;
    int n_batch;
    const int* info;
    hipStream_t stream;
    int nsplit;
    double* split_buf; int64_t split_stride;
    int dma_ok;
    int skip_reduce;
    int small64;
    int bn, bz_div;
    int64_t bstride;
};
__device__ __forceinline__ void gemm_block_z(const GemmArgs& g, int z, int* tb, int* item) {
    if (g.bn > 1) { *tb = z / g.bz_div; *item = z - *tb * g.bz_div; }
    else { *tb = 0; *item = z; }
}
__device__ __forceinline__ bool gemm_block_order(const GemmArgs& g, int* bx, int* tb, int* item) {
    if (g.bn > 1) {
        const int lin = (int)blockIdx.x + (int)gridDim.x * (int)blockIdx.z;
        const int rest = lin / g.bn;
        *tb = lin - rest * g.bn;
        *bx = rest / g.bz_div;
        *item = rest - *bx * g.bz_div;
        return true;
    }
    *bx = (int)blockIdx.x; *tb = 0; *item = (int)blockIdx.z;
    return true;
}
static inline unsigned gemm_grid_z(const GemmArgs& g) { return (unsigned)(g.bz_div * g.bn); }
static inline void gemm_fill_batch(const gpry_ctx* ctx, GemmArgs* g) {
    g->bn = ctx->bn; g->bstride = ctx->bstride; g->bz_div = g->batch ? g->n_batch : 1;
}
struct GemmPart { int bz, ti, tj, lo, hi, slice; };
struct GemmRedTile { int bz, ti, tj, nslice; };
struct GemmPartsPlan {
    GemmPart* d_parts = nullptr; int* d_first = nullptr; GemmRedTile* d_red = nullptr;
    int nwg = 0, nred = 0, max_slices = 0;
};
struct GemmShape { int M, N, K; };
int gemm_parts_segment(int kmode, int lower_only, const std::vector<GemmShape>& shapes, int slots);
int gemm_parts_plan_build(gpry_ctx* ctx, int kmode, int lower_only, const std::vector<GemmShape>& items, int seg_pairs,
                          GemmPartsPlan* out);
void gemm_parts_plan_free(GemmPartsPlan* pl);
int gemm_dma_parts_launch(gpry_ctx* ctx, const GemmArgs& g, bool a_trans, bool b_trans, int epi, const GemmPartsPlan& pl,
                          int64_t slice_stride);
int gemm_f64_launch(gpry_ctx* ctx, const GemmArgs& g, bool a_trans, bool b_trans, int epi);
int gemm64_launch(gpry_ctx* ctx, const GemmArgs& g, bool a_trans, bool b_trans, int epi);
int gemm_split_scratch(gpry_ctx* ctx, int nsplit, int64_t slice, double** buf);
int launch_trtri_diag(gpry_ctx* ctx, const double* L, double* V, int64_t Np, hipStream_t st, bool zero_right = false);
int ensure_pred_xs(gpry_ctx* ctx);
int launch_point_full(gpry_ctx* ctx, const double* x, int want_kinv, double* kstar, double* G, double* u, double* part,
                      double* mean_part, double* ss_part, double* out);
int launch_trtri_diag128(gpry_ctx* ctx, const double* L, double* V, int64_t Np, hipStream_t st, bool clear_right);
int launch_trtri_diag_range(gpry_ctx* ctx, const double* L, double* V, int64_t Np, int blk0, int nblk, hipStream_t st);
bool gemm_dma_usable(const GemmArgs& g, int M, int N, int K);
int gemm_dma_launch_product(gpry_ctx* ctx, const GemmArgs& g, bool a_trans, bool b_trans, int epi, dim3 grid);
int sweep_gemm_dma_sp_launch(gpry_ctx* ctx, const GemmArgs& g);

int upload_params(gpry_ctx* ctx, const double* theta);
int launch_scale_train(gpry_ctx* ctx);
int launch_kernel_train(gpry_ctx* ctx, double* K, int add_noise, double* U = nullptr);
int launch_kernel_rows(gpry_ctx* ctx, int64_t row0, int k, int64_t ldk, double* Bk, double* Cb);
int launch_cross_build(gpry_ctx* ctx, const double* Xc, int64_t m0, int64_t mc,
                       int64_t ldk, double* Kst, double* mean_part, int raw_affine,
                       hipStream_t st = nullptr);
int launch_cross_prepare(gpry_ctx* ctx);
int launch_cross_build_mfma(gpry_ctx* ctx, const double* Xc, int64_t m0, int64_t mc, int64_t ldk, double* Kst, double* mean_part,
                            int raw_affine, int hybrid = 0);
int launch_cross_mean_bound(gpry_ctx* ctx, const double* Xc, int64_t m0, int64_t mc, double* mean_part, double* sabs_part,
                            double ubnd, double uhi, unsigned long long* live_cnt);
int launch_cross_build_small(gpry_ctx* ctx, const double* Xc, int64_t m0, int64_t mc, int64_t ldk,
                             double* Kst, double* mean_part, int raw_affine);
int launch_predict_mean_small(gpry_ctx* ctx, const double* Xc, int64_t M, int nsplit, double* part_out);
int launch_gates(gpry_ctx* ctx, const double* Xc, int64_t M, uint8_t* mask);
int launch_predict_small_std(gpry_ctx* ctx, const double* Xc, int M, double* kstar, double* mean_part,
                             double* ss_part);
int launch_gradx(gpry_ctx* ctx, const double* x, int raw_affine, int want_kinv, double* kstar, double* G,
                 double* u, double* w, double* part, double* out);
int launch_gradx_batch(gpry_ctx* ctx, const double* Xb, int64_t m, int raw_affine, const double* Wm, int64_t ldw,
                       double* out);
int launch_lml_small(gpry_ctx* ctx, int want_grad, double* out, int* info);
int launch_lml_small_batch(gpry_ctx* ctx, int B, const double* params, int want_grad, double* out, int* info);
int launch_lml_traces(gpry_ctx* ctx, const double* Kinv, const double* alpha,
                      double* grad_out_dev, const double* lq_dev, double* host_res, int info_at);

int potrf_lower_fused(gpry_ctx* ctx, double* A, int64_t Np);
int potrf_lower_overlap(gpry_ctx* ctx, double* A, int64_t Np);
int potrf_stacked(gpry_ctx* ctx, double* A, double* U, int64_t Np);
bool potrf_stacked_usable(const gpry_ctx* ctx, int64_t Np);
int transpose_upper_launch(gpry_ctx* ctx, const double* U, double* V, int64_t Np);
int trtri_lower(gpry_ctx* ctx, const double* L, double* V, double* T, int64_t Np);
int trtri_pipeline_begin(gpry_ctx* ctx, const double* L, double* V, double* T, int64_t Np);
int trtri_pipeline_step(gpry_ctx* ctx, int blocks_done);
int trtri_pipeline_finish(gpry_ctx* ctx);
void trtri_pipeline_abort(gpry_ctx* ctx);
void trtri_pipe_free(gpry_ctx* ctx);
int lauum_lower(gpry_ctx* ctx, const double* V, double* Kinv, int64_t Np);
int factor_chain_slices(gpry_ctx* ctx, int64_t Np, int* slices);
int solve_alpha(gpry_ctx* ctx, const double* V, const double* y, double* z, double* alpha,
                int64_t Np);
int logdet_and_quad(gpry_ctx* ctx, const double* L, const double* z, int64_t Np,
                    double* out2_dev, double* host_res, int info_at);
int rocsolver_potrf_trtri(gpry_ctx* ctx, double* A, double* V, int64_t Np, int want_v);

int require_model(gpry_ctx* ctx, bool need_factor);
int serve_stop(gpry_ctx* ctx);
void serve_free(gpry_ctx* ctx);
void serve_stats(gpry_ctx* ctx, int64_t* launches, int64_t* requests);
int serve_predict_mean(gpry_ctx* ctx, const double* X, int64_t M, double* part, int* nsplit_out, unsigned* gate_bits);
#define GPRY_SERVE_MAXM 8

int build_factor(gpry_ctx* ctx, double* A, double* V, double* T, int* info_host);
constexpr int LML_RES_INFO = 2 + GPRY_THETA_MAX;
int lml_chain(gpry_ctx* ctx, int want_grad, double* dres);
bool panel_timed_out(int marker);
int panel_timeout_error(gpry_ctx* ctx, int marker);
int loo_pass_launch(gpry_ctx* ctx, const double* V, double* qpart, double* wpart);
int pv_panel_launch(gpry_ctx* ctx, const double* dX, int64_t npts, int64_t cols, double* Kst, int64_t ldk);
int lml_hess_km_launch(gpry_ctx* ctx, double* Km);
struct BatchChain {
    const char* name;
    int (*chain)(gpry_ctx* ctx, int want_grad, double* dres);
    bool latency_only;
    int64_t part_min, split_min;
    int head, info_at;
    double (*value)(const double* row);
};
int objective_batch_general(gpry_ctx* ctx, const BatchChain& bc, const double* thetas, int64_t B, int want_grad, double* value,
                            double* grad, int* info);

int objective_entry(gpry_ctx* ctx, const char* name, const double* thetas, int64_t B);
static inline void note_xs_foreign(gpry_ctx* ctx, bool had) { if (had && ctx->factor_valid) ctx->xs_foreign = true; }
struct ThetaScope {
    gpry_ctx* c; bool had; double saved[GPRY_THETA_MAX];
    ThetaScope(gpry_ctx* ctx, const double* theta) : c(ctx), had(ctx->have_theta) {
        memcpy(saved, ctx->theta, sizeof(saved));
        for (int k = 0; k < ctx_ntheta(ctx); k++) ctx->theta[k] = theta[k];
        ctx->have_theta = true;
    }
    ~ThetaScope() { memcpy(c->theta, saved, sizeof(saved)); c->have_theta = had; }
    void factor_chain_ran() { note_xs_foreign(c, had); }
};
static inline void objective_row_unwritten(double* row, int info_at) { row[info_at] = -1.0; row[info_at + 1] = -1.0; }
int objective_row(gpry_ctx* ctx, int64_t bytes, int info_at, double** hres, double** dres);
int objective_status(gpry_ctx* ctx, const char* name, int64_t which, const double* row, int info_at, int* info);
int objective_wait(gpry_ctx* ctx, const char* name, int rc, const double* row, int info_at, int* info);
void objective_write(const gpry_ctx* ctx, int info, double head, const double* g, const double* h, double* value, double* grad,
                     double* hess);
static inline double lml_head(const double* row) { return -0.5 * row[1] - row[0]; }

static inline int dp_class(int d) { return d <= 4 ? 4 : d <= 8 ? 8 : d <= 16 ? 16 : d <= 24 ? 24 : 32; }
static inline int splitk_count(int64_t tiles, int64_t Np) {
    int nsplit = 1;
    while (nsplit < 4 && tiles * nsplit * 2 <= 1100 && Np / (nsplit * 2) >= 256) nsplit *= 2;
    return nsplit;
}

int ensure_capacity(gpry_ctx* ctx, int64_t N, int d);
int ensure_pinned(gpry_ctx* ctx, int64_t bytes);
```

gpry_amd/csrc/ctx.hip:

```cpp
#include "common.h"
#include <string>
#include <stdarg.h>
#include <dlfcn.h>

thread_local char g_last_error[1024] = {0};
void trtri_plan_free(gpry_ctx* ctx);
void overlap_plan_free(gpry_ctx* ctx);

int gpry_fail(gpry_ctx* ctx, int code, const char* fmt, ...) {
    va_list ap;
    va_start(ap, fmt);
    vsnprintf(g_last_error, sizeof(g_last_error), fmt, ap);
    va_end(ap);
    if (ctx) { strncpy(ctx->err, g_last_error, sizeof(ctx->err) - 1); }
    return code;
}

template <typename T>
int dev_alloc(gpry_ctx* ctx, T** p, int64_t count) {
    *p = nullptr;
    if (count <= 0) count = 1;
    HIP_TRY(ctx, hipMalloc((void**)p, sizeof(T) * (size_t)count));
    return 0;
}
// ... 125 lines not shown
    }
    if (ctx->dpw && 2 * Np < ctx->pw_np) {
        (void)hipStreamSynchronize(ctx->stream);
        (void)hipFree(ctx->dpw);
        ctx->dpw = nullptr; ctx->pw_cap = 0; ctx->pw_np = 0;
    }
    if (ctx->dvtg && 2 * (2 + (int64_t)d) * Np * Np < ctx->vtg_cap) {
        (void)hipStreamSynchronize(ctx->stream);
        (void)hipFree(ctx->dvtg);
        ctx->dvtg = nullptr; ctx->vtg_cap = 0;
    }
    ctx->N = N; ctx->Np = Np; ctx->d = d; ctx->dpad = dpad;
    return 0;
}

extern "C" {

int gpry_version(void) { return 100; }

int gpry_device_count(int* n) {
    int c = 0;
    hipError_t e = hipGetDeviceCount(&c);
    if (e != hipSuccess) { *n = 0; return gpry_fail(nullptr, -2, "hipGetDeviceCount: %s", hipGetErrorString(e)); }
    *n = c;
    return 0;
}

int gpry_device_info(int device, char* name, int name_len, int64_t* hbm_bytes, int* n_cu,
                     int* clock_khz, char* arch, int arch_len) {
    hipDeviceProp_t p;
    hipError_t e = hipGetDeviceProperties(&p, device);
    if (e != hipSuccess) return gpry_fail(nullptr, -2, "hipGetDeviceProperties: %s", hipGetErrorString(e));
    if (name && name_len > 0) { strncpy(name, p.name, name_len - 1); name[name_len - 1] = 0; }
    if (arch && arch_len > 0) { strncpy(arch, p.gcnArchName, arch_len - 1); arch[arch_len - 1] = 0; }
    if (hbm_bytes) *hbm_bytes = (int64_t)p.totalGlobalMem;
    if (n_cu) *n_cu = p.multiProcessorCount;
    if (clock_khz) *clock_khz = p.clockRate;
    return 0;
}

int gpry_ctx_create(int device, gpry_ctx** out) {
    if (!out) return gpry_fail(nullptr, -1, "gpry_ctx_create: out is NULL");
    *out = nullptr;
    hipError_t e = hipSetDevice(device);
    if (e != hipSuccess) return gpry_fail(nullptr, -2, "hipSetDevice(%d): %s", device, hipGetErrorString(e));
    gpry_ctx* ctx = new gpry_ctx();
    ctx->device = device;
    memset(&ctx->tf, 0, sizeof(ctx->tf));
    ctx->tf.y_std = 1.0; ctx->tf.clip_hi = INFINITY;
    e = hipStreamCreateWithFlags(&ctx->stream, hipStreamNonBlocking);
    if (e != hipSuccess) { delete ctx; return gpry_fail(nullptr, -2, "hipStreamCreate: %s", hipGetErrorString(e)); }
    e = hipStreamCreateWithFlags(&ctx->stream2, hipStreamNonBlocking);
    if (e != hipSuccess) { delete ctx; return gpry_fail(nullptr, -2, "hipStreamCreate: %s", hipGetErrorString(e)); }
    if (hipMalloc((void**)&ctx->dinfo, 16 * sizeof(int)) != hipSuccess) { delete ctx; return gpry_fail(nullptr, -2, "hipMalloc info"); }
    (void)hipMemset(ctx->dinfo, 0, 16 * sizeof(int));
    if (const char* env = getenv("GPRY_HIP_OPTIONS")) {
        std::string all(env);
        size_t pos = 0;
        while (pos < all.size()) {
            size_t end = all.find(',', pos);
            if (end == std::string::npos) end = all.size();
            const std::string item = all.substr(pos, end - pos);
            pos = end + 1;
            if (item.empty()) continue;
            const size_t eq = item.find('=');
            char* tail = nullptr;
            const long long v = eq == std::string::npos ? 0 : strtoll(item.c_str() + eq + 1, &tail, 10);
            if (eq == std::string::npos || eq == 0 || tail == item.c_str() + eq + 1 || *tail != '\0' ||
                gpry_ctx_set_option(ctx, item.substr(0, eq).c_str(), (int64_t)v) != 0) {
                (void)gpry_ctx_destroy(ctx);
                return gpry_fail(nullptr, -1, "GPRY_HIP_OPTIONS: bad entry '%s'", item.c_str());
            }
        }
    }
    *out = ctx;
    return 0;
}

int gpry_ctx_destroy(gpry_ctx* ctx) {
    if (!ctx) return 0;
    (void)hipSetDevice(ctx->device);
    (void)hipStreamSynchronize(ctx->stream);
    if (ctx->stream2) (void)hipStreamSynchronize(ctx->stream2);
    timers_collect(ctx);
    serve_free(ctx);
    trtri_plan_free(ctx);
    trtri_pipe_free(ctx);
    overlap_plan_free(ctx);
    void* bufs[] = {ctx->dX, ctx->dXs, ctx->dy, ctx->dnoise, ctx->dA, ctx->dV, ctx->dW, ctx->dW2, ctx->dW3,
                    ctx->dalpha_, ctx->dvec, ctx->dinfo, ctx->dparams, ctx->dXc, ctx->dmask, ctx->dy_all,
                    ctx->dsig_all, ctx->dacq_all, ctx->dKst, ctx->dpart, ctx->dkeys, ctx->dhist, ctx->dselp,
                    ctx->dcand, ctx->dsel, ctx->dU, ctx->dXkb, ctx->dkbout, ctx->pr.dXc, ctx->pr.dmask,
                    ctx->pr.dy, ctx->pr.dsig, ctx->pr.dacq, ctx->dG,
                    ctx->gate_sv, ctx->gate_coef, ctx->gate_trust, ctx->dsplit, ctx->dbord, ctx->barena, ctx->dXcs, ctx->dYcs,
                    ctx->dub, ctx->dXg, ctx->dgidx, ctx->snap.dV, ctx->snap.dalpha_, ctx->snap.dXs, ctx->snap.dX, ctx->dmc, ctx->dknn,
                    ctx->dph, ctx->djoint, ctx->dloo, ctx->dsvm, ctx->dhess, ctx->dtg, ctx->dpw, ctx->dvtg};
    for (void* b : bufs) if (b) (void)hipFree(b);
    if (ctx->hpin) (void)hipHostFree(ctx->hpin);
    if (ctx->hloo) (void)hipHostFree(ctx->hloo);
    if (ctx->hsvm) (void)hipHostFree(ctx->hsvm);
    if (ctx->hbres) (void)hipHostFree(ctx->hbres);
    (void)hipStreamDestroy(ctx->stream);
    if (ctx->stream2) (void)hipStreamDestroy(ctx->stream2);
    for (hipEvent_t ev : ctx->ev_pool) (void)hipEventDestroy(ev);
    for (hipStream_t st : ctx->tp_streams) (void)hipStreamDestroy(st);
    for (hipEvent_t ev : ctx->tp_events) (void)hipEventDestroy(ev);
    delete ctx;
    return 0;
}

const char* gpry_last_error(gpry_ctx* ctx) { return ctx ? ctx->err : g_last_error; }

int gpry_ctx_sync(gpry_ctx* ctx) {
    if (!ctx) return gpry_fail(nullptr, -1, "gpry_ctx_sync: ctx is NULL");
    HIP_TRY(ctx, hipStreamSynchronize(ctx->stream));
    return 0;
}

namespace {
struct OptionSpec {
    const char* key;
    int64_t lo, hi;
    int64_t (*get)(const gpry_ctx*);
    void (*set)(gpry_ctx*, int64_t);
};
#define OPT_INT(KEY, FIELD, LO, HI, AFTER)                                                         \
    {KEY, LO, HI, [](const gpry_ctx* c) -> int64_t { return (int64_t)c->FIELD; },                  \
     [](gpry_ctx* c, int64_t v) { c->FIELD = (decltype(c->FIELD))v; AFTER; }}
const int64_t BIG = (int64_t)1 << 40;
const OptionSpec OPTIONS[] = {
    OPT_INT("timing", opt_timing, 0, 1, (void)0),
    OPT_INT("chol", opt_chol, 0, 1, c->lml_cache = false),
    OPT_INT("chol_overlap", opt_chol_overlap, 0, 1, c->lml_cache = false),
    OPT_INT("factor_pipeline", opt_factor_pipeline, 0, 1, (void)0),
    OPT_INT("factor_pipeline_min", opt_factor_pipeline_min, 0, BIG, (void)0),
    OPT_INT("gemm_dma", opt_gemm_dma, 0, 1, (void)0),
    OPT_INT("gemm_streamk", opt_gemm_streamk, 0, BIG, trtri_plan_free(c)),
    OPT_INT("gemm_small", opt_gemm_small, 0, BIG, c->lml_cache = false),
    OPT_INT("cross_mfma", opt_cross_mfma, 0, 1, (void)0),
    OPT_INT("cross_hybrid", opt_cross_hybrid, 0, 1, (void)0),
    OPT_INT("sweep_chunk", opt_sweep_chunk, 0, BIG, c->opt_sweep_chunk = round_up(c->opt_sweep_chunk, 1024)),
    OPT_INT("topk_host", opt_topk_host, 0, BIG, (void)0),
    OPT_INT("lml_small", opt_lml_small, 0, 1, c->lml_cache = false),
    OPT_INT("lml_cache", opt_lml_cache, 0, 1, c->lml_cache = false),
    OPT_INT("lml_batch", opt_lml_batch, 0, BIG, (void)0),
    OPT_INT("lml_batch_mb", opt_lml_batch_mb, 1, BIG, (void)0),
    OPT_INT("lml_schedule", opt_lml_schedule, 0, 1, (void)0),
    OPT_INT("lml_streams", opt_lml_streams, 1, 8, (void)0),
    OPT_INT("chol_tp_segments", opt_chol_tp_segments, 0, 1, c->lml_cache = false),
    OPT_INT("panel_debug", opt_panel_debug, 0, 511, c->lml_cache = false),
    OPT_INT("tp_left", opt_tp_left, 0, 1, (void)0),
    OPT_INT("tp_block", opt_tp_block, 128, BIG, c->opt_tp_block = round_up(c->opt_tp_block, 128); overlap_plan_free(c)),
    OPT_INT("tp_tail", opt_tp_tail, 128, BIG, c->opt_tp_tail = round_up(c->opt_tp_tail, 128); overlap_plan_free(c)),
    OPT_INT("predict_small", opt_predict_small, 0, BIG, (void)0),
    OPT_INT("predict_split", opt_predict_split, 0, 1, (void)0),
    OPT_INT("sweep_upload", opt_sweep_upload, 0, 1, (void)0),
    OPT_INT("sweep_overlap", opt_sweep_overlap, 0, 1, (void)0),
    OPT_INT("sweep_prune", opt_sweep_prune, 0, 1, (void)0),
    OPT_INT("sweep_mean_bound", opt_sweep_mean_bound, 0, 1, (void)0),
    OPT_INT("sweep_screen", opt_sweep_screen, 0, 1, (void)0),
    OPT_INT("sweep_small_map", opt_sweep_small_map, 0, 1, (void)0),
    OPT_INT("select_fused", opt_select_fused, 0, 1, (void)0),
    OPT_INT("prune_one_select", opt_prune_one_select, 0, 1, (void)0),
    OPT_INT("chol_stacked", opt_chol_stacked, 0, BIG, c->lml_cache = false),
    OPT_INT("chol_stacked_dense", opt_chol_stacked_dense, 0, 1, c->lml_cache = false),
    OPT_INT("predict_gates", opt_predict_gates, 0, 1, (void)0),
    OPT_INT("predict_serve", opt_predict_serve, 0, 1, (void)0),
    OPT_INT("serve_idle_us", opt_serve_idle_us, 10, 1000000, (void)0),
    OPT_INT("mcmc_mapped", opt_mcmc_mapped, 0, 1, (void)0),
    OPT_INT("kb_rank", opt_kb_rank, 0, 1, (void)0),
    OPT_INT("svm_iters_per_launch", opt_svm_iters, 1, BIG, (void)0),
};
#undef OPT_INT
const OptionSpec* find_option(const char* key) {
    for (const OptionSpec& o : OPTIONS) if (!strcmp(o.key, key)) return &o;
    return nullptr;
}
}

int gpry_ctx_set_option(gpry_ctx* ctx, const char* key, int64_t value) {
    if (!ctx || !key) return gpry_fail(ctx, -1, "gpry_ctx_set_option: NULL argument");
    GPRY_TRY(serve_stop(ctx));
    const OptionSpec* o = find_option(key);
    if (!o) return gpry_fail(ctx, -1, "unknown option '%s'", key);
    if (value < o->lo || value > o->hi)
        return gpry_fail(ctx, -1, "%s must be in %lld..%lld (got %lld)", key, (long long)o->lo, (long long)o->hi, (long long)value);
    o->set(ctx, value);
    return 0;
}

int gpry_ctx_get_option(gpry_ctx* ctx, const char* key, int64_t* value) {
    if (!ctx || !key || !value) return gpry_fail(ctx, -1, "gpry_ctx_get_option: NULL argument");
    const OptionSpec* o = find_option(key);
    if (!o) return gpry_fail(ctx, -1, "unknown option '%s'", key);
    *value = o->get(ctx);
    return 0;
}

int gpry_set_train(gpry_ctx* ctx, const double* X_, const double* y_, const double* alpha,
                   int64_t N, int d) {
    if (!ctx) return gpry_fail(nullptr, -1, "gpry_set_train: ctx is NULL");
    GPRY_TRY(serve_stop(ctx));
    if (N <= 0 || d <= 0) return gpry_fail(ctx, -1, "set_train: need N > 0 and d > 0 (got %lld, %d)", (long long)N, d);
    if (d > GPRY_MAX_DIM) return gpry_fail(ctx, -1, "set_train: d=%d > GPRY_MAX_DIM=%d is not supported by this build", d, GPRY_MAX_DIM);
    if (!X_ || !y_ || !alpha) return gpry_fail(ctx, -1, "set_train: X_, y_ and alpha must not be NULL");
    HIP_TRY(ctx, hipSetDevice(ctx->device));
    if (d != ctx->d) { ctx->sw_M = 0; ctx->sw_pruned = 0; }
    GPRY_TRY(ensure_capacity(ctx, N, d));
    hipStream_t st = ctx->stream;
    for (int k = 0; k < d; k++) {
        double s = 0.0, lo = X_[k], hi = X_[k];
        for (int64_t i = 0; i < N; i++) {
            const double v = X_[i * d + k];
            s += v;
            lo = v < lo ? v : lo; hi = v > hi ? v : hi;
        }
        ctx->xsum[k] = s;
        ctx->xcenter[k] = s / (double)N;
// ... 341 lines not shown
```

gpry_amd/csrc/gemm_dma.hip:

```cpp
#include "common.h"
#include <algorithm>

#include "gemm_dma_body.h"

template <bool AT, bool BT, int EPI>
__global__ __launch_bounds__(256, 2) void gemm_dma_kernel(GemmArgs g) {
    constexpr int A_SZ = !AT ? KC_DOUBLES : MC_DOUBLES, B_SZ = BT ? KC_DOUBLES : MC_DOUBLES;
    __shared__ __attribute__((aligned(16))) double smem[2 * (A_SZ + B_SZ)];
    int bx, tb, bz;
    if (!gemm_block_order(g, &bx, &tb, &bz)) return;
    gemm_dma_tile_body<AT, BT, EPI>(g, smem, bx, (int)blockIdx.y, bz, nullptr, tb);
}

bool gemm_dma_usable(const GemmArgs& g, int M, int N, int K) {
    if (M <= 0 || N <= 0 || K < 32) return false;
    if (M % BM || N % BN || K % 32) return false;
    if ((g.lda | g.ldb | g.ldc) & 1) return false;
    return true;
}

template <bool AT, bool BT>
static int gd_launch_epi(gpry_ctx* ctx, const GemmArgs& g, int epi, dim3 grid) {
    hipStream_t st = g.stream ? g.stream : ctx->stream;
    switch (epi) {
        case EPI_STORE: hipLaunchKernelGGL((gemm_dma_kernel<AT, BT, EPI_STORE>), grid, dim3(256), 0, st, g); break;
        case EPI_STORE_NEG: hipLaunchKernelGGL((gemm_dma_kernel<AT, BT, EPI_STORE_NEG>), grid, dim3(256), 0, st, g); break;
        case EPI_SUB: hipLaunchKernelGGL((gemm_dma_kernel<AT, BT, EPI_SUB>), grid, dim3(256), 0, st, g); break;
        default: return gpry_fail(ctx, -1, "gemm_dma: bad epilogue %d", epi);
    }
    HIP_TRY(ctx, hipGetLastError());
    return 0;
}

int gemm_dma_launch_product(gpry_ctx* ctx, const GemmArgs& g0, bool a_trans, bool b_trans, int epi, dim3 grid) {
    GemmArgs g = g0;
    gemm_fill_batch(ctx, &g);
    grid.z = gemm_grid_z(g);
    if ((g.tile_map & 15) == TM_ROWMAJOR) {
        g.tile_map = TM_BALANCED;
        const int tm = g.M / BM, tn = g.N / BN;
        if (g.lower_only && tm == tn && g.batch == nullptr) grid.x = (unsigned)(tm * (tm + 1) / 2);
    }
    if (!a_trans && !b_trans) return gd_launch_epi<false, false>(ctx, g, epi, grid);
    if (!a_trans && b_trans) return gd_launch_epi<false, true>(ctx, g, epi, grid);
    if (a_trans && !b_trans) return gd_launch_epi<true, false>(ctx, g, epi, grid);
    return gpry_fail(ctx, -1, "gemm_dma: the TT layout is not built");
}

template <bool AT, bool BT, int EPI>
__global__ __launch_bounds__(256, 2) void gemm_dma_parts_kernel(GemmArgs g, const GemmPart* __restrict__ parts,
                                                                const int* __restrict__ first) {
    constexpr int A_SZ = !AT ? KC_DOUBLES : MC_DOUBLES, B_SZ = BT ? KC_DOUBLES : MC_DOUBLES;
    __shared__ __attribute__((aligned(16))) double smem[2 * (A_SZ + B_SZ)];
    const int p1 = first[blockIdx.x + 1];
    for (int p = first[blockIdx.x]; p < p1; p++) {
        const GemmPart pt = parts[p];
        gemm_dma_tile_body<AT, BT, EPI>(g, smem, 0, 0, 0, &pt, (int)blockIdx.z);
        asm volatile("s_waitcnt vmcnt(0) lgkmcnt(0)" ::: "memory");
        __syncthreads();
    }
}

__global__ __launch_bounds__(256) void gemm_parts_reduce_kernel(GemmArgs g, const GemmRedTile* __restrict__ tiles, double sign) {
    const int tb = (int)blockIdx.z;
    if (g.info != nullptr && *bset(g.info, tb, g.bstride) != 0) return;
    const GemmRedTile t = tiles[blockIdx.x];
    const double* split_buf = bset(g.split_buf, tb, g.bstride);
    double* Cb = bset(g.C, tb, g.bstride);
    int64_t coff = 0;
    if (g.batch != nullptr) coff = g.batch[t.bz].c_off;
    const int row0 = t.ti * BM, col0 = t.tj * BN;
    const int rbeg = (int)blockIdx.y * (BM / 8);
    for (int e = threadIdx.x; e < (BM / 8) * (BN / 2); e += 256) {
        const int rr = rbeg + e / (BN / 2), cc = (e % (BN / 2)) * 2;
        const int64_t off = coff + (int64_t)(row0 + rr) * g.ldc + col0 + cc;
        double2 acc = make_double2(0.0, 0.0);
        for (int sidx = 0; sidx < t.nslice; sidx++) {
            const double2 v = *reinterpret_cast<const double2*>(split_buf + (int64_t)sidx * g.split_stride + off);
            acc.x += v.x; acc.y += v.y;
        }
        *reinterpret_cast<double2*>(Cb + off) = make_double2(sign * acc.x, sign * acc.y);
    }
}

namespace {
struct HostTile { int ti, tj, pairs; };
void enumerate_tiles(int kmode, int lower_only, const GemmShape& it, std::vector<HostTile>& out) {
    out.clear();
    const int tm = it.M / BM, tn = it.N / BN;
    for (int ti = 0; ti < tm; ti++)
        for (int tj = 0; tj < tn; tj++) {
            if (lower_only && tj > ti) continue;
            const int row0 = ti * BM, col0 = tj * BN;
            int kbeg = 0, kend = it.K;
            if (kmode == KM_A_LOWER) kend = std::min(it.K, row0 + BM);
            else if (kmode == KM_B_LOWER) kbeg = std::min(it.K, col0);
            else if (kmode == KM_AT_LOWER_B_LOWER) kbeg = std::min(it.K, std::max(row0, col0));
            else if (kmode == KM_B_UPPER) kend = std::min(it.K, col0 + BN);
            else if (kmode == KM_AT_LOWER) kbeg = std::min(it.K, row0);
            out.push_back({ti, tj, (kend - kbeg) / (2 * BK)});
        }
    std::stable_sort(out.begin(), out.end(), [](const HostTile& a, const HostTile& b) { return a.pairs > b.pairs; });
}
}

int gemm_parts_segment(int kmode, int lower_only, const std::vector<GemmShape>& shapes, int slots) {
    int64_t total = 0;
    std::vector<HostTile> tl;
    for (const GemmShape& it : shapes) {
        enumerate_tiles(kmode, lower_only, it, tl);
// ... 96 lines not shown
```

gpry_amd/csrc/gemm_dma_body.h:

```cpp
#pragma once
#include "common.h"

#define BM 128
#define BN 128
#define BK 16
#define SMC 144
#define KC_DOUBLES 2048
#define MC_DOUBLES 2304
#define KC_MI_BYTES (16 * 16 * 8)
#define MC_KSTEP_BYTES (4 * SMC * 8)

typedef const __attribute__((address_space(1))) void* gptr_t;
typedef __attribute__((address_space(3))) void* lptr_t;

__device__ __forceinline__ void gd_dma16(const double* g, double* l) {
    __builtin_amdgcn_global_load_lds((gptr_t)g, (lptr_t)l, 16, 0, 0);
}

struct GdFrag { double a0, a1, a2, a3, b0, b1, b2, b3; };

template <bool AKC, bool BKC, int BUF, int KK>
__device__ __forceinline__ void gd_load_frag(GdFrag& f, unsigned addrA, unsigned addrB) {
    constexpr int a_sz = (AKC ? KC_DOUBLES : MC_DOUBLES) * 8, b_sz = (BKC ? KC_DOUBLES : MC_DOUBLES) * 8;
    constexpr int buf_all = BUF * (a_sz + b_sz);
// ... 15 lines not shown
}
template <int NPEND>
__device__ __forceinline__ void gd_wait_frag(GdFrag& f) {
    asm volatile("s_waitcnt lgkmcnt(%8)"
                 : "+v"(f.a0), "+v"(f.a1), "+v"(f.a2), "+v"(f.a3), "+v"(f.b0), "+v"(f.b1), "+v"(f.b2), "+v"(f.b3)
                 : "n"(NPEND) : "memory");
}
__device__ __forceinline__ void gd_mma_frag(v4d (&acc)[4][4], const GdFrag& f) {
    const double a[4] = {f.a0, f.a1, f.a2, f.a3};
    const double b[4] = {f.b0, f.b1, f.b2, f.b3};
#pragma unroll
    for (int mi = 0; mi < 4; mi++)
#pragma unroll
        for (int ni = 0; ni < 4; ni++)
            acc[mi][ni] = __builtin_amdgcn_mfma_f64_16x16x4f64(a[mi], b[ni], acc[mi][ni], 0, 0, 0);
}
__device__ __forceinline__ void gd_mma_row(v4d (&acc)[4][4], const GdFrag& f, int mi) {
    const double a = mi == 0 ? f.a0 : mi == 1 ? f.a1 : mi == 2 ? f.a2 : f.a3;
    acc[mi][0] = __builtin_amdgcn_mfma_f64_16x16x4f64(a, f.b0, acc[mi][0], 0, 0, 0);
    acc[mi][1] = __builtin_amdgcn_mfma_f64_16x16x4f64(a, f.b1, acc[mi][1], 0, 0, 0);
    acc[mi][2] = __builtin_amdgcn_mfma_f64_16x16x4f64(a, f.b2, acc[mi][2], 0, 0, 0);
    acc[mi][3] = __builtin_amdgcn_mfma_f64_16x16x4f64(a, f.b3, acc[mi][3], 0, 0, 0);
}

template <bool AT, bool BT, int EPI>
__device__ __forceinline__ void gemm_dma_tile_body(const GemmArgs& g, double* smem, const int bx, const int by, const int bz_,
                                                   const GemmPart* part = nullptr, const int tb = 0) {
    const int bz = part ? part->bz : bz_;
    constexpr bool AKC = !AT, BKC = BT;
    constexpr int A_SZ = AKC ? KC_DOUBLES : MC_DOUBLES, B_SZ = BKC ? KC_DOUBLES : MC_DOUBLES;
    constexpr int BUF_SZ = A_SZ + B_SZ;
    if (g.info != nullptr && *bset(g.info, tb, g.bstride) != 0) return;

    double* const C0 = bset(g.C, tb, g.bstride);
    double* const split0 = bset(g.split_buf, tb, g.bstride);
    const double* A = bset(g.A, tb, g.bstride); const double* B = bset(g.B, tb, g.bstride); double* C = C0;
    int M = g.M, N = g.N, K = g.K;
    if (g.batch != nullptr) {
        GemmBatchItem it = g.batch[bz];
        A += it.a_off; B += it.b_off; C += it.c_off;
        M = it.M; N = it.N; K = it.K;
    }
    const int tiles_m = M / BM, tiles_n = N / BN;
    int ti, tj;
    if (part) { ti = part->ti; tj = part->tj; }
    else {
        const int b = bx;
        if ((g.tile_map & 15) == TM_SWEEP) {
            const int a = (g.tile_map >> 4) & 15, c = 6 - a;
            const int nsi = (tiles_m + (1 << a) - 1) >> a, nsj = (tiles_n + (1 << c) - 1) >> c;
            const int xcd = b & 7, q = b >> 3;
            const int s = (q >> 6) * 8 + xcd, within = q & 63;
            if (s >= nsi * nsj) return;
            const int si = nsi - 1 - s / nsj, sj = s % nsj;
            ti = (si << a) + (within >> c);
            tj = (sj << c) + (within & ((1 << c) - 1));
        } else if ((g.tile_map & 15) == TM_BALANCED) {
            if (g.lower_only && tiles_m == tiles_n) {
                int i = (int)((sqrt(8.0 * (double)b + 1.0) - 1.0) * 0.5);
                while ((i + 1) * (i + 2) / 2 <= b) i++;
                while (i * (i + 1) / 2 > b) i--;
                ti = i; tj = b - i * (i + 1) / 2;
                if (ti >= tiles_m) return;
            } else if (g.kmode == KM_B_LOWER || g.kmode == KM_B_UPPER) {
                tj = b / tiles_m;
                ti = b - tj * tiles_m;
                if (g.kmode == KM_B_UPPER) tj = tiles_n - 1 - tj;
            } else {
                ti = b / tiles_n;
                tj = b - ti * tiles_n;
                if (g.kmode == KM_A_LOWER) ti = tiles_m - 1 - ti;
            }
        } else {
            ti = b / tiles_n;
            tj = b - ti * tiles_n;
        }
        if (ti < 0 || tj < 0 || ti >= tiles_m || tj >= tiles_n) return;
        if (g.lower_only && tj > ti) return;
    }
    const int row0 = ti * BM, col0 = tj * BN;
    int kbeg = 0, kend = K;
    if (g.kmode == KM_A_LOWER) kend = min(K, row0 + BM);
    else if (g.kmode == KM_B_LOWER) kbeg = min(K, col0);
    else if (g.kmode == KM_AT_LOWER_B_LOWER) kbeg = min(K, max(row0, col0));
    else if (g.kmode == KM_B_UPPER) kend = min(K, col0 + BN);
    else if (g.kmode == KM_AT_LOWER) kbeg = min(K, row0);
    bool partial = g.nsplit > 1;
    if (part) {
        kend = kbeg + part->hi * 2 * BK;
        kbeg = kbeg + part->lo * 2 * BK;
        partial = part->slice >= 0;
        if (partial) C = split0 + (int64_t)part->slice * g.split_stride + (C - C0);
    } else if (g.nsplit > 1) {
        const int all = (kend - kbeg) / (2 * BK);
        const int per = (all + g.nsplit - 1) / g.nsplit;
        const int lo = min(all, by * per), hi = min(all, lo + per);
        kend = kbeg + hi * 2 * BK;
        kbeg = kbeg + lo * 2 * BK;
        C = split0 + (int64_t)by * g.split_stride + (C - C0);
    }
    const int nslab = (kend - kbeg) / BK;

    const int lane = threadIdx.x & 63, wave = threadIdx.x >> 6;
    const int wr = wave >> 1, wc = wave & 1;
    const int r = lane & 15, gq = lane >> 4;

    double* const cbase = C + (int64_t)(row0 + wr * 64 + gq) * g.ldc + col0 + wc * 64 + r;
    v4d acc[4][4];
    if (EPI == EPI_SUB && !partial) {
#pragma unroll
        for (int i = 0; i < 4; i++)
#pragma unroll
            for (int j = 0; j < 4; j++)
#pragma unroll
                for (int q = 0; q < 4; q++) acc[i][j][q] = -cbase[(int64_t)(i * 16 + 4 * q) * g.ldc + j * 16];
    } else {
#pragma unroll
        for (int i = 0; i < 4; i++)
#pragma unroll
            for (int j = 0; j < 4; j++) acc[i][j] = (v4d){0.0, 0.0, 0.0, 0.0};
    }

    if (nslab > 0) {
    const double* srcA[4];
    const double* srcB[4];
#pragma unroll
    for (int j = 0; j < 4; j++) {
        const int q = wave * 4 + j;
        const int row = q * 8 + (lane >> 3), pp = lane & 7;
        const int p = pp ^ ((row >> 1) & 7);
        srcA[j] = AKC ? A + (int64_t)(row0 + row) * g.lda + kbeg + 2 * p
                      : A + (int64_t)(kbeg + q) * g.lda + row0 + 2 * lane;
        srcB[j] = BKC ? B + (int64_t)(col0 + row) * g.ldb + kbeg + 2 * p
                      : B + (int64_t)(kbeg + q) * g.ldb + col0 + 2 * lane;
    }
    const int64_t stepA = AKC ? BK : (int64_t)BK * g.lda, stepB = BKC ? BK : (int64_t)BK * g.ldb;
    auto issue_piece = [&](int s, int buf, int j) {
        double* As = smem + buf * BUF_SZ;
        double* Bs = As + A_SZ;
        if (j < 4) gd_dma16(srcA[j] + s * stepA, As + (AKC ? (wave * 4 + j) * 128 : (wave * 4 + j) * SMC));
        else gd_dma16(srcB[j - 4] + s * stepB, Bs + (BKC ? (wave * 4 + j - 4) * 128 : (wave * 4 + j - 4) * SMC));
    };
    auto issue = [&](int s, int buf) {
#pragma unroll
        for (int j = 0; j < 8; j++) issue_piece(s, buf, j);
    };

    const unsigned smem_base = (unsigned)(uintptr_t)(lptr_t)smem;
    unsigned addrA[4], addrB[4];
#pragma unroll
    for (int kk = 0; kk < 4; kk++) {
        addrA[kk] = AKC ? smem_base + (wr * 64 + r) * 128 + 16 * ((((gq >> 1) ^ (r >> 1)) & 7) ^ (2 * kk)) + 8 * (gq & 1)
                        : smem_base + gq * (SMC * 8) + (wr * 64 + r) * 8;
        addrB[kk] = BKC ? smem_base + (wc * 64 + r) * 128 + 16 * ((((gq >> 1) ^ (r >> 1)) & 7) ^ (2 * kk)) + 8 * (gq & 1)
                        : smem_base + gq * (SMC * 8) + (wc * 64 + r) * 8;
    }

    issue(0, 0);
    issue(1, 1);
    asm volatile("s_waitcnt vmcnt(8)" ::: "memory");
    __builtin_amdgcn_s_barrier();
    __builtin_amdgcn_sched_barrier(0);

    GdFrag f0, f1;
    gd_load_frag<AKC, BKC, 0, 0>(f0, addrA[0], addrB[0]);

#define GD_SLAB_STEP(BUF, S)                                                                 \
    {                                                                                        \
        gd_load_frag<AKC, BKC, BUF, 1>(f1, addrA[1], addrB[1]);                              \
        gd_wait_frag<8>(f0);                                                                 \
        __builtin_amdgcn_sched_barrier(0);                                                   \
        gd_mma_frag(acc, f0);                                                                \
        __builtin_amdgcn_sched_barrier(0);                                                   \
        gd_load_frag<AKC, BKC, BUF, 2>(f0, addrA[2], addrB[2]);                              \
        gd_wait_frag<8>(f1);                                                                 \
        __builtin_amdgcn_sched_barrier(0);                                                   \
        gd_mma_frag(acc, f1);                                                                \
        __builtin_amdgcn_sched_barrier(0);                                                   \
        gd_load_frag<AKC, BKC, BUF, 3>(f1, addrA[3], addrB[3]);                              \
        gd_wait_frag<8>(f0);                                                                 \
        __builtin_amdgcn_sched_barrier(0);                                                   \
        gd_mma_frag(acc, f0);                                                                \
        __builtin_amdgcn_sched_barrier(0);                                                   \
          \
        asm volatile("s_waitcnt vmcnt(0)" ::: "memory");                                     \
        gd_wait_frag<0>(f1);                                                                 \
        __builtin_amdgcn_s_barrier();                                                        \
        __builtin_amdgcn_sched_barrier(0);                                                   \
          \
        const int s2 = min((S) + 2, nslab - 1);                                              \
        gd_mma_row(acc, f1, 0);                                                              \
        __builtin_amdgcn_sched_barrier(0);                                                   \
        gd_load_frag<AKC, BKC, (BUF) ^ 1, 0>(f0, addrA[0], addrB[0]);                        \
        issue_piece(s2, BUF, 0); issue_piece(s2, BUF, 1);                                    \
        __builtin_amdgcn_sched_barrier(0);                                                   \
        gd_mma_row(acc, f1, 1);                                                              \
        __builtin_amdgcn_sched_barrier(0);                                                   \
        issue_piece(s2, BUF, 2); issue_piece(s2, BUF, 3); issue_piece(s2, BUF, 4);           \
        __builtin_amdgcn_sched_barrier(0);                                                   \
        gd_mma_row(acc, f1, 2);                                                              \
        __builtin_amdgcn_sched_barrier(0);                                                   \
        issue_piece(s2, BUF, 5); issue_piece(s2, BUF, 6); issue_piece(s2, BUF, 7);           \
        __builtin_amdgcn_sched_barrier(0);                                                   \
        gd_mma_row(acc, f1, 3);                                                              \
        __builtin_amdgcn_sched_barrier(0);                                                   \
    }
    for (int s = 0; s < nslab; s += 2) {
        GD_SLAB_STEP(0, s)
        GD_SLAB_STEP(1, s + 1)
    }
#undef GD_SLAB_STEP
    asm volatile("s_waitcnt vmcnt(0) lgkmcnt(0)" ::: "memory");
    }

#pragma unroll
    for (int mi = 0; mi < 4; mi++)
#pragma unroll
        for (int ni = 0; ni < 4; ni++)
#pragma unroll
            for (int q = 0; q < 4; q++) {
                double* p = cbase + (int64_t)(mi * 16 + 4 * q) * g.ldc + ni * 16;
                const double v = acc[mi][ni][q];
                if (EPI == EPI_STORE || partial) *p = v;
                else *p = -v;
            }
}
```

gpry_amd/gpr.py:

```python
import copy
import os
import sys
import warnings
from collections.abc import Mapping
from numbers import Number

import numpy as np
import scipy.optimize

from gpry_amd import _lib
from gpry_amd.kernels import RBF, Matern, ConstantKernel as C, clone
from gpry_amd.preprocessing import DummyPreprocessor, Normalize_bounds, Normalize_y
from gpry_amd.svm import SVM
from gpry_amd.tools import (check_random_state, delta_logp_of_1d_nstd, generic_params_names,
                            get_Xnumber, is_in_bounds, shrink_bounds)

try:
    from sklearn.base import BaseEstimator as _BE, RegressorMixin as _RM
except Exception:
    _BE = _RM = object


_LAUNCHERS = (("WORLD_SIZE", ("RANK", "LOCAL_RANK")),
              ("OMPI_COMM_WORLD_SIZE", ("OMPI_COMM_WORLD_RANK", "OMPI_COMM_WORLD_LOCAL_RANK")),
              ("PMI_SIZE", ("PMI_RANK", "MPI_LOCALRANKID")),
              ("SLURM_STEP_NUM_TASKS", ("SLURM_PROCID",)))
_WORLD_SIZE_VARS = tuple(v for v, _ in _LAUNCHERS)
_LOCAL_RANK_VARS = ("LOCAL_RANK", "OMPI_COMM_WORLD_LOCAL_RANK", "MPI_LOCALRANKID", "SLURM_LOCALID")
_LAUNCH_NOTE = {"said": False}


def multi_process_launch():
    for size_var, rank_vars in _LAUNCHERS:
        try:
            many = int(os.environ.get(size_var, "1")) > 1
        except ValueError:
            many = False
        if not many:
            continue
        if any(os.environ.get(v, "") != "" for v in rank_vars):
            return True
        if not _LAUNCH_NOTE["said"]:
            _LAUNCH_NOTE["said"] = True
            import logging
            logging.getLogger("gpry_amd").info(
                "%s=%s without %s: treated as ONE process that may use every visible GPU, not as a rank of a "
                "multi-process launch", size_var, os.environ.get(size_var), " / ".join(rank_vars))
    mpi = sys.modules.get("mpi4py.MPI")
    try:
        return mpi is not None and mpi.Is_initialized() and mpi.COMM_WORLD.Get_size() > 1
    except Exception:
        return False


_FIT_CONTEXT_OPTIONS = ("chol", "chol_overlap", "chol_stacked", "factor_pipeline", "factor_pipeline_min", "gemm_dma", "gemm_streamk",
                        "gemm_small", "lml_small", "lml_cache", "lml_batch", "lml_batch_mb", "lml_schedule", "lml_streams",
                        "tp_block", "tp_tail")


def copy_fit_options(src, dst):
    if not (hasattr(src, "get_option") and hasattr(dst, "set_option")):
        return
    for key in _FIT_CONTEXT_OPTIONS:
        try:
            v = src.get_option(key)
            if dst.get_option(key) != v:
                dst.set_option(key, v)
        except Exception:
            pass


def default_device_index():
    for var in ("GPRY_HIP_DEVICE",) + _LOCAL_RANK_VARS:
        if os.environ.get(var, "") != "":
            n, idx = _lib.device_count(), int(os.environ[var])
            if n > 0 and idx >= n:
                if n == 1 and any(os.environ.get(v, "") != "" for v in
                                  ("HIP_VISIBLE_DEVICES", "ROCR_VISIBLE_DEVICES", "CUDA_VISIBLE_DEVICES")):
                    return 0
                if os.environ.get("GPRY_HIP_DEVICE_WRAP", "") == "1":
                    return idx % n
                raise _lib.GpryHipError(
                    f"{var}={idx} but only {n} GPU(s) are visible: one process per GPU "
                    "(set GPRY_HIP_DEVICE_WRAP=1 to share devices, without RCCL)")
            return idx
    return 0


def fit_contexts():
    try:
        return max(1, int(os.environ.get("GPRY_HIP_FIT_CONTEXTS", "3")))
    except ValueError:
        return 3


_BATCH_GROUP_MIN_RUNS = 3


def batch_contexts(n_train=None):
    env = os.environ.get("GPRY_HIP_FIT_BATCH_CONTEXTS", "")
    if env != "":
        try:
            return max(1, int(env))
        except ValueError:
            pass
    if n_train is None:
        return 2
    return 1 if n_train <= 300 else 3


def fit_schedule(n_train, n_runs):
    env = os.environ.get("GPRY_HIP_FIT_SCHEDULE", "auto").lower()
    try:
        tp_groups = max(1, int(os.environ.get("GPRY_HIP_FIT_TP_GROUPS", "1")))
    except ValueError:
        tp_groups = 1
    if env == "latency":
        return "latency", None
    if env != "throughput":
        npad = -(-int(n_train) // 128) * 128
        if npad < 2304 or n_runs < 6:
            return "latency", None
    return "throughput", tp_groups


def fit_context_devices(own, n_restarts, spec=None):
    per = fit_contexts()
    if spec is None:
        env = os.environ.get("GPRY_HIP_DEVICES", "").strip().lower()
        if env not in ("", "none", "1", "all"):
            devs = [int(v) for v in env.split(",")]
        elif env in ("none", "1") or (env == "" and multi_process_launch()):
            devs = [own]
        else:
            n = _lib.device_count()
            devs = list(range(n)) if n > 1 else [own]
        devs = [own] + [v for v in dict.fromkeys(devs) if v != own]
        spec = [devs[i % len(devs)] for i in range(per * len(devs))]
# ... 1285 lines not shown
```

include/gpry_hip.h:

```cpp
#ifndef GPRY_HIP_H
#define GPRY_HIP_H

#include <stdint.h>

#ifdef __cplusplus
extern "C" {
#endif

typedef struct gpry_ctx gpry_ctx;
typedef struct gpry_comm gpry_comm;
typedef struct gpry_group gpry_group;

enum { GPRY_RBF = 0, GPRY_MATERN12 = 1, GPRY_MATERN32 = 2, GPRY_MATERN52 = 3 };
#define GPRY_KERNEL_WHITE 0x10

#define GPRY_MAX_DIM 32

typedef struct {
    int has_x_affine;
    double x_lo[GPRY_MAX_DIM];
    double x_span[GPRY_MAX_DIM];
    double y_mean, y_std;
    double clip_hi;
} gpry_affine;
// ... 136 lines not shown
int64_t gpry_var_theta_grad_panel(gpry_ctx* ctx);

int gpry_predict_grad(gpry_ctx* ctx, const double* x, int want_kinv, double* kgrad,
                      double* mean_grad, double* kinvk_grad);

int gpry_predict_grad_batch(gpry_ctx* ctx, const double* X, int64_t m, int want_kinv, double* mean,
                            double* std, double* mean_grad, double* kinvk_grad);

int gpry_predict_point(gpry_ctx* ctx, const double* x, int mask_bits, int want_kinv, double* mean, double* std,
                       double* mean_grad, double* kinvk_grad, int* verdict);

int gpry_set_gates(gpry_ctx* ctx, const double* sv, const double* coef, int64_t n_sv, double gamma,
                   double intercept, int positive_is_finite, const double* trust_bounds);

int gpry_svm_fit(gpry_ctx* ctx, const double* X, const uint8_t* finite, int64_t N, int64_t d, double C, double gamma,
                 double eps, int64_t max_iter, double* alpha, double* rho, double* objective, double* violation,
                 int64_t* n_iter, int* status, double* device_ms);

int gpry_sweep_logexp(gpry_ctx* ctx, const double* X, int64_t M, const uint8_t* mask,
                      double zeta, double baseline, double sigma_n,
                      double* y_all, double* sigma_all, double* acq_all,
                      int64_t* n_nan);
int gpry_sweep_logexp_given(gpry_ctx* ctx, const double* X, int64_t M, const uint8_t* mask,
                            const double* y_given, const double* sigma_given,
                            double zeta, double baseline, double sigma_n,
                            double* y_all, double* sigma_all, double* acq_all,
                            int64_t* n_nan);
int gpry_sweep_info(gpry_ctx* ctx, int* panel_form, double* est);
int gpry_sweep_fetch(gpry_ctx* ctx, int64_t M, double* y_all, double* sigma_all, double* acq_all);
int gpry_sweep_topk(gpry_ctx* ctx, int64_t Kp, const int64_t* exclude, int64_t n_exclude,
                    gpry_cand* top, int64_t* n_out, double* bound);
int gpry_sweep_prune_info(gpry_ctx* ctx, int64_t* info, double* dinfo);
int gpry_sweep_screen_info(gpry_ctx* ctx, int64_t out[2]);

int gpry_kb_reset(gpry_ctx* ctx);
int gpry_kb_register(gpry_ctx* ctx, const double* X, int64_t m, int64_t* first,
                     double* var0);
int gpry_kb_gram(gpry_ctx* ctx, int64_t p, double* G, double* kvec, int64_t* n);
int gpry_kb_gram_rows(gpry_ctx* ctx, const int64_t* p, int64_t n_rows, double* G, double* kvec, int64_t* n);
int gpry_kb_rank(gpry_ctx* ctx, const double* X_new, int64_t m_new, double* var0, int64_t n_session,
                 const int64_t* idx, const double* y, const double* sigma, const double* acq, int64_t n_offer,
                 const int64_t* order, int64_t n_order, const double* params, int64_t n_points,
                 int64_t* slot_idx, double* slot_y, double* slot_sigma, double* slot_acq, double* slot_acq_cond,
                 int64_t* cache_counter, int64_t* info, int64_t* stats);

int gpry_comm_unique_id(uint8_t id[128]);
int gpry_comm_init(gpry_ctx* ctx, int world, int rank, const uint8_t id[128],
                   gpry_comm** out);
int gpry_comm_destroy(gpry_comm* comm);
int gpry_comm_info(gpry_comm* comm, int* world, int* rank, int* device);
int gpry_comm_allgather(gpry_comm* comm, const void* send, int64_t bytes, void* recv);
int gpry_comm_allreduce_max(gpry_comm* comm, double* inout, int64_t n);
int gpry_comm_barrier(gpry_comm* comm);

int gpry_group_create(int n, const int* devices, gpry_ctx* adopt0, gpry_group** out);
int gpry_group_destroy(gpry_group* group);
int gpry_group_size(gpry_group* group, int* n, int* transport);
gpry_ctx* gpry_group_member(gpry_group* group, int i);
const char* gpry_group_last_error(gpry_group* group);
int gpry_group_set_model(gpry_group* group, const double* X_, const double* y_, const double* alpha,
                         int64_t N, int d, int kernel_id, const double* theta, const gpry_affine* tf,
                         int* info);
int gpry_group_set_gates(gpry_group* group, const double* sv, const double* coef, int64_t n_sv,
                         double gamma, double intercept, int positive_is_finite,
                         const double* trust_bounds);
int gpry_group_sweep_logexp(gpry_group* group, const double* X, int64_t M, const uint8_t* mask,
                            double zeta, double baseline, double sigma_n, double* y_all,
                            double* sigma_all, double* acq_all, int64_t* n_nan);
int gpry_group_sweep_logexp_given(gpry_group* group, const double* X, int64_t M, const uint8_t* mask,
                                  const double* y_given, const double* sigma_given,
                                  double zeta, double baseline, double sigma_n, double* y_all,
                                  double* sigma_all, double* acq_all, int64_t* n_nan);
int gpry_group_sweep_fetch(gpry_group* group, int64_t M, double* y_all, double* sigma_all,
                           double* acq_all);
int gpry_group_sweep_topk(gpry_group* group, int64_t Kp, const int64_t* exclude, int64_t n_exclude,
                          gpry_cand* top, int64_t* n_out, double* bound, int* exhausted);
int gpry_group_lml_batch(gpry_group* group, const double* thetas, int n_theta, int want_grad,
                         double* lml, double* grad, int* info);

int gpry_timing_reset(gpry_ctx* ctx);
int gpry_timing_get(gpry_ctx* ctx, const char* name, double* total_ms, int64_t* count);
int gpry_microbench(gpry_ctx* ctx, int kind, int64_t bytes, double* value);

int gpry_debug_gemm(gpry_ctx* ctx, const double* A, const double* B, double* C, int M, int N,
                    int K, int a_trans, int b_trans, int epi, int kmode, int lower_only,
                    int tile_map);

int gpry_debug_logexp(gpry_ctx* ctx, const double* mu, const double* sigma, int64_t n, double zeta,
                      double baseline, double sigma_n, double* acq);

#ifdef __cplusplus
}
#endif
#endif
```

Baseline: 68.03 million.

## Add row-block triangular inverse and incremental K^-1 accumulation pipeline

Adds a row-block variant of the lower-triangular inverse, used by default when Np is between rows_min and the stream-K limit. It processes blocks of rows in sequence, each with a recursive diagonal tree plus panel GEMMs, and pipelines the blocks on a side stream behind the Cholesky panels. An optional path (kinv_rows, off by default) builds K^-1 row block by row block on a third stream through a new accumulating GEMM epilogue, in place of a separate LAUUM. This adds plan state, streams, events and a debug scratch accessor, and the new schedule may expose less parallelism than the previous phase-based one.

```diff
diff --git a/gpry_amd/_lib.py b/gpry_amd/_lib.py
--- a/gpry_amd/_lib.py
+++ b/gpry_amd/_lib.py
@@ -146,6 +146,7 @@
     "gpry_timing_get": (C.c_int, [_vp, C.c_char_p, _P(C.c_double), _P(C.c_int64)]),
     "gpry_sweep_info": (C.c_int, [_vp, _P(C.c_int), _vp]),
     "gpry_microbench": (C.c_int, [_vp, C.c_int, C.c_int64, _P(C.c_double)]),
+    "gpry_debug_lml_scratch": (C.c_int, [_vp, C.c_int, _vp]),
     "gpry_debug_gemm": (C.c_int, [_vp, _vp, _vp, _vp] + [C.c_int] * 9),
     "gpry_debug_logexp": (C.c_int, [_vp, _vp, _vp, C.c_int64, C.c_double, C.c_double, C.c_double, _vp]),
 }
@@ -1001,6 +1002,11 @@
                                               int(lower_only), int(tile_map)), "gpry_debug_gemm")
         return Cout
 
+    def debug_lml_scratch(self, which):
+        out = np.empty((self.N, self.N))
+        self._check(self._lib.gpry_debug_lml_scratch(self._h, int(which), _ptr(out)), "gpry_debug_lml_scratch")
+        return out
+
     def debug_logexp(self, mu, sigma, zeta, baseline, sigma_n):
         mu, sigma = _f64(mu), _f64(sigma)
         acq = np.empty(len(mu))
diff --git a/gpry_amd/csrc/api.hip b/gpry_amd/csrc/api.hip
--- a/gpry_amd/csrc/api.hip
+++ b/gpry_amd/csrc/api.hip
@@ -70,7 +70,7 @@
 
 int build_factor(gpry_ctx* ctx, double* A, double* V, double* T, int* info_host) {
     GPRY_TRY(launch_scale_train(ctx));
-    const bool want_stacked = ctx->opt_chol != 1 && potrf_stacked_usable(ctx, ctx->Np);
+    const bool want_stacked = ctx->opt_chol != 1 && potrf_stacked_usable(ctx, ctx->Np) && !factor_rows_apply(ctx, ctx->Np);
     {
         StageScope s(ctx, "kernel_build");
         GPRY_TRY(launch_kernel_train(ctx, A, 1, want_stacked ? T : nullptr));
@@ -85,7 +85,7 @@
             ~PipeGuard() { if (armed) trtri_pipeline_abort(c); }
         } guard{ctx};
         if (ctx->opt_factor_pipeline && ctx->opt_chol == 0 && ctx->Np >= ctx->opt_factor_pipeline_min && ctx->bn == 1 && !ctx->tp &&
-            !potrf_stacked_usable(ctx, ctx->Np)) {
+            !want_stacked) {
             const int rc = trtri_pipeline_begin(ctx, A, V, T, ctx->Np);
             if (rc < 0) return rc;
             piped = rc == 0;
@@ -126,7 +126,12 @@
 constexpr int RES_INFO = LML_RES_INFO;
 static_assert(RES_INFO + 3 <= GPRY_BRES_STRIDE, "result row too short");
 int lml_chain(gpry_ctx* ctx, int want_grad, double* dres) {
-    GPRY_TRY(build_factor(ctx, ctx->dW, ctx->dW2, ctx->dW3, nullptr));
+    const bool kinv_rows = want_grad && kinv_rows_apply(ctx, ctx->Np);
+    ctx->kinv_from_row = 0;
+    ctx->chain_kinv = kinv_rows ? ctx->dW3 : nullptr;
+    const int frc = build_factor(ctx, ctx->dW, ctx->dW2, ctx->dW3, nullptr);
+    ctx->chain_kinv = nullptr;
+    GPRY_TRY(frc);
     double* dz = ctx->dvec;
     double* da = ctx->dvec + ctx->Np;
     double* dout = ctx->dvec + 2 * ctx->Np;
@@ -138,7 +143,8 @@
     if (!want_grad) return 0;
     {
         StageScope s(ctx, "lauum");
-        GPRY_TRY(lauum_lower(ctx, ctx->dW2, ctx->dW3, ctx->Np));
+        if (kinv_rows) GPRY_TRY(kinv_rows_finish(ctx, ctx->dW2, ctx->dW3, ctx->Np));
+        else GPRY_TRY(lauum_lower(ctx, ctx->dW2, ctx->dW3, ctx->Np));
     }
     StageScope s(ctx, "lml_traces");
     return launch_lml_traces(ctx, ctx->dW3, da, dout + 2, dout, dres, RES_INFO);
@@ -1023,6 +1029,18 @@
 
 }
 
+extern "C" int gpry_debug_lml_scratch(gpry_ctx* ctx, int which, double* out) {
+    if (!ctx || !out) return gpry_fail(ctx, -1, "gpry_debug_lml_scratch: NULL argument");
+    if (which < 0 || which > 2) return gpry_fail(ctx, -1, "gpry_debug_lml_scratch: which must be 0 (L), 1 (V) or 2 (K^-1)");
+    if (ctx->N <= 0) return gpry_fail(ctx, -1, "gpry_debug_lml_scratch: no training set");
+    HIP_TRY(ctx, hipSetDevice(ctx->device));
+    const double* src = which == 0 ? ctx->dW : which == 1 ? ctx->dW2 : ctx->dW3;
+    HIP_TRY(ctx, hipMemcpy2DAsync(out, sizeof(double) * ctx->N, src, sizeof(double) * ctx->Np, sizeof(double) * ctx->N, (size_t)ctx->N,
+                                  hipMemcpyDeviceToHost, ctx->stream));
+    HIP_TRY(ctx, hipStreamSynchronize(ctx->stream));
+    return 0;
+}
+
 extern "C" int gpry_debug_gemm(gpry_ctx* ctx, const double* A, const double* B, double* C, int M, int N,
                                int K, int a_trans, int b_trans, int epi, int kmode, int lower_only,
                                int tile_map) {
diff --git a/gpry_amd/csrc/chol.hip b/gpry_amd/csrc/chol.hip
--- a/gpry_amd/csrc/chol.hip
+++ b/gpry_amd/csrc/chol.hip
@@ -48,8 +48,26 @@
     int blocks_done = 0, diag_lo = 0, diag_hi = 0;
     std::vector<TrtriPhaseLevel> levels;
 };
+struct RowsLevel { int64_t first = 0; int n = 0, mM = 0, mN = 0, aligned = 0; };
+struct RowsBlock {
+    int r0 = 0, r1 = 0;
+    std::vector<RowsLevel> levels;
+    GemmPartsPlan sk_w, sk_v;
+};
+struct RowsPlan {
+    int b = 0;
+    std::vector<RowsBlock> blocks;
+    GemmBatchItem* d_items = nullptr;
+    int max_slices = 0;
+    void release() {
+        for (auto& bl : blocks) { gemm_parts_plan_free(&bl.sk_w); gemm_parts_plan_free(&bl.sk_v); }
+        if (d_items) (void)hipFree(d_items);
+        *this = RowsPlan();
+    }
+};
 struct TrtriPlan {
     int64_t Np = 0;
+    RowsPlan rows;
     int leaf = 1;
     std::vector<GemmBatchItem*> d_t, d_v;
     std::vector<int> count, maxM, maxN;
@@ -68,6 +86,7 @@
         for (auto& q : sk_v) gemm_parts_plan_free(&q);
         for (auto& ph : phases) for (auto& pv : ph.levels) { gemm_parts_plan_free(&pv.sk_t); gemm_parts_plan_free(&pv.sk_v); }
         gemm_parts_plan_free(&sk_lauum);
+        rows.release();
     }
 };
 void trtri_plan_free(gpry_ctx* ctx) {
@@ -78,14 +97,76 @@
     ctx->trtri_plan = nullptr;
 }
 
+bool factor_rows_apply(const gpry_ctx* ctx, int64_t Np) {
+    return ctx->opt_trtri_rows > 0 && ctx->opt_chol == 0 && !ctx->tp && Np >= 256 && Np >= ctx->opt_rows_min && Np <= ctx->opt_gemm_streamk;
+}
+static int64_t kinv_rows_width(const gpry_ctx* ctx) {
+    return ctx->opt_kinv_rows > 1 ? ctx->opt_kinv_rows : ctx->opt_trtri_rows > 0 ? ctx->opt_trtri_rows : 512;
+}
+bool kinv_rows_apply(const gpry_ctx* ctx, int64_t Np) {
+    return ctx->opt_kinv_rows > 0 && ctx->opt_gemm_dma && ctx->opt_chol == 0 && !ctx->tp && Np >= 256 && Np >= ctx->opt_rows_min &&
+           Np <= ctx->opt_gemm_streamk;
+}
+
+static int rows_plan_build(gpry_ctx* ctx, int64_t Np, int b, int slots, RowsPlan* out) {
+    out->release();
+    std::vector<GemmBatchItem> all;
+    for (int64_t r0 = 0; r0 < Np; r0 += b) {
+        RowsBlock bl;
+        bl.r0 = (int)r0; bl.r1 = (int)std::min<int64_t>(r0 + b, Np);
+        std::vector<TriNode> nodes;
+        const int nlev = build_tree(bl.r0 / 64, bl.r1 / 64, nodes);
+        for (int lev = 1; lev <= nlev; lev++) {
+            RowsLevel rl; rl.aligned = 1;
+            std::vector<GemmBatchItem> bt, bv;
+            for (auto& nd : nodes) {
+                if (nd.level != lev) continue;
+                const int64_t lo = nd.lo * 64, mid = nd.mid * 64, hi = nd.hi * 64;
+                const int m = (int)(hi - mid), n = (int)(mid - lo);
+                bt.push_back({mid * Np + lo, lo * Np + lo, mid * Np + lo, m, n, n, 0});
+                bv.push_back({mid * Np + mid, mid * Np + lo, mid * Np + lo, m, n, m, 0});
+                if (m > rl.mM) rl.mM = m;
+                if (n > rl.mN) rl.mN = n;
+                if (m % 128 || n % 128) rl.aligned = 0;
+            }
+            rl.n = (int)bt.size(); rl.first = (int64_t)all.size();
+            all.insert(all.end(), bt.begin(), bt.end());
+            all.insert(all.end(), bv.begin(), bv.end());
+            bl.levels.push_back(rl);
+        }
+        out->blocks.push_back(bl);
+    }
+    for (auto& bl : out->blocks) {
+        if (bl.r0 == 0) continue;
+        const int m = bl.r1 - bl.r0;
+        const std::vector<GemmShape> sw = {{m, bl.r0, bl.r0}}, sv = {{m, bl.r0, m}};
+        int rc = gemm_parts_plan_build(ctx, KM_B_LOWER, 0, sw, gemm_parts_segment(KM_B_LOWER, 0, sw, slots), &bl.sk_w);
+        if (rc == 0) rc = gemm_parts_plan_build(ctx, KM_A_LOWER, 0, sv, gemm_parts_segment(KM_A_LOWER, 0, sv, slots), &bl.sk_v);
+        if (rc) { out->release(); return rc; }
+        out->max_slices = std::max(out->max_slices, std::max(bl.sk_w.max_slices, bl.sk_v.max_slices));
+    }
+    if (!all.empty()) {
+        hipError_t e = hipMalloc(&out->d_items, all.size() * sizeof(GemmBatchItem));
+        if (e == hipSuccess) e = hipMemcpy(out->d_items, all.data(), all.size() * sizeof(GemmBatchItem), hipMemcpyHostToDevice);
+        if (e != hipSuccess) { out->release(); return gpry_fail(ctx, -2, "row-block plan (Np = %lld): %s", (long long)Np, hipGetErrorString(e)); }
+    }
+    out->b = b;
+    return 0;
+}
+
 static int trtri_plan_get(gpry_ctx* ctx, int64_t Np, TrtriPlan** out) {
     if (!ctx->trtri_plan) ctx->trtri_plan = new TrtriPlan();
     TrtriPlan& pl = *static_cast<TrtriPlan*>(ctx->trtri_plan);
-    if (pl.Np == Np) { *out = &pl; return 0; }
+    int slots = 512;
+    { hipDeviceProp_t prop; if (hipGetDeviceProperties(&prop, ctx->device) == hipSuccess && prop.multiProcessorCount > 0) slots = 2 * prop.multiProcessorCount; }
+    if (pl.Np == Np) {
+        if (factor_rows_apply(ctx, Np) && pl.rows.b != (int)ctx->opt_trtri_rows)
+            GPRY_TRY(rows_plan_build(ctx, Np, (int)ctx->opt_trtri_rows, slots, &pl.rows));
+        *out = &pl;
+        return 0;
+    }
     pl.release();
     pl = TrtriPlan();
-    int slots = 512;
-    { hipDeviceProp_t prop; if (hipGetDeviceProperties(&prop, ctx->device) == hipSuccess && prop.multiProcessorCount > 0) slots = 2 * prop.multiProcessorCount; }
     pl.leaf = (Np > 128 && Np <= 1024) ? 2 : 1;
     std::vector<TriNode> nodes;
     int nlev = build_tree(0, (int)(Np / (64 * pl.leaf)), nodes);
@@ -214,6 +295,10 @@
             return gpry_fail(ctx, -2, "trtri plan (Np = %lld): %s", (long long)Np, hipGetErrorString(e));
         }
     }
+    if (factor_rows_apply(ctx, Np)) {
+        const int rc = rows_plan_build(ctx, Np, (int)ctx->opt_trtri_rows, slots, &pl.rows);
+        if (rc) { pl.release(); pl = TrtriPlan(); return rc; }
+    }
     pl.Np = Np;
     *out = &pl;
     return 0;
@@ -280,8 +365,80 @@
     for (int64_t i = (int64_t)blockIdx.x * blockDim.x + threadIdx.x; i < n2; i += stride) p[i] = make_double2(0.0, 0.0);
 }
 
+static int kinv_rows_update(gpry_ctx* ctx, const double* V, double* Kinv, int64_t Np, int64_t r0, int64_t r1, hipStream_t st) {
+    GemmArgs g = {};
+    g.A = V + r0 * Np; g.lda = Np; g.B = V + r0 * Np; g.ldb = Np; g.C = Kinv; g.ldc = Np;
+    g.M = (int)r1; g.N = (int)r1; g.K = (int)(r1 - r0); g.kshift = (int)r0;
+    g.kmode = KM_AT_LOWER_B_LOWER; g.lower_only = 1; g.tile_map = TM_ROWMAJOR; g.info = ctx->dinfo; g.stream = st;
+    const int tm = (int)(r1 / 128);
+    return gemm_dma_launch_product(ctx, g, true, false, EPI_ACC, dim3((unsigned)(tm * (tm + 1) / 2), 1, 1));
+}
+int kinv_rows_finish(gpry_ctx* ctx, const double* V, double* Kinv, int64_t Np) {
+    const int64_t bk = kinv_rows_width(ctx);
+    for (int64_t r0 = ctx->kinv_from_row; r0 < Np; r0 += bk)
+        GPRY_TRY(kinv_rows_update(ctx, V, Kinv, Np, r0, std::min(r0 + bk, Np), ctx->stream));
+    ctx->kinv_from_row = 0;
+    return 0;
+}
+static bool rows_chain_kinv(const gpry_ctx* ctx, const RowsPlan& rp, const double* T) {
+    return ctx->chain_kinv != nullptr && ctx->chain_kinv == T && kinv_rows_width(ctx) == rp.b;
+}
+static int rows_stage(gpry_ctx* ctx, const RowsPlan& rp, const double* L, double* V, double* T, int64_t Np, size_t i, hipStream_t st,
+                      hipStream_t kst = nullptr, hipEvent_t evk = nullptr) {
+    const RowsBlock& bl = rp.blocks[i];
+    const int64_t slice = (int64_t)rp.b * Np;
+    GPRY_TRY(launch_trtri_diag_range(ctx, L, V, Np, bl.r0 / 64, (bl.r1 - bl.r0) / 64, st));
+    for (const RowsLevel& rl : bl.levels)
+        GPRY_TRY(trtri_level_products(ctx, L, V, T, Np, 1, rl.aligned, rp.d_items + rl.first, rl.n, rl.mM, rl.mN,
+                                      rp.d_items + rl.first + rl.n, rl.n, rl.mM, rl.mN, st));
+    if (i > 0) {
+        GemmArgs h = {};
+        h.A = V + (int64_t)bl.r0 * Np + bl.r0; h.lda = Np; h.B = T + (int64_t)bl.r0 * Np; h.ldb = Np; h.C = V + (int64_t)bl.r0 * Np; h.ldc = Np;
+        h.M = bl.r1 - bl.r0; h.N = bl.r0; h.K = bl.r1 - bl.r0;
+        h.kmode = KM_A_LOWER; h.info = ctx->dinfo; h.stream = st;
+        GPRY_TRY(gemm_dma_parts_launch(ctx, h, false, false, EPI_STORE_NEG, bl.sk_v, slice));
+    }
+    const bool kinv_here = i + 1 < rp.blocks.size() && rows_chain_kinv(ctx, rp, T);
+    if (kinv_here && kst != nullptr && kst != st) {
+        HIP_TRY(ctx, hipEventRecord(evk, st));
+        HIP_TRY(ctx, hipStreamWaitEvent(kst, evk, 0));
+        GPRY_TRY(kinv_rows_update(ctx, V, T, Np, bl.r0, bl.r1, kst));
+    }
+    if (i + 1 < rp.blocks.size()) {
+        const RowsBlock& nx = rp.blocks[i + 1];
+        GemmArgs g = {};
+        g.A = L + (int64_t)nx.r0 * Np; g.lda = Np; g.B = V; g.ldb = Np; g.C = T + (int64_t)nx.r0 * Np; g.ldc = Np;
+        g.M = nx.r1 - nx.r0; g.N = nx.r0; g.K = nx.r0;
+        g.kmode = KM_B_LOWER; g.info = ctx->dinfo; g.stream = st;
+        GPRY_TRY(gemm_dma_parts_launch(ctx, g, false, false, EPI_STORE, nx.sk_w, slice));
+        if (kinv_here && (kst == nullptr || kst == st)) GPRY_TRY(kinv_rows_update(ctx, V, T, Np, bl.r0, bl.r1, st));
+    } else if (rows_chain_kinv(ctx, rp, T)) ctx->kinv_from_row = bl.r0;
+    return 0;
+}
+static int rows_clear_and_reserve(gpry_ctx* ctx, const RowsPlan& rp, double* V, int64_t Np, hipStream_t st) {
+    double* sbuf = nullptr;
+    if (rp.max_slices > 0) GPRY_TRY(gemm_split_scratch(ctx, rp.max_slices, (int64_t)rp.b * Np, &sbuf));
+    if (ctx->bn > 1) {
+        const int64_t n2 = Np * Np / 2;
+        int64_t nb = (n2 + 2047) / 2048;
+        if (nb > 4096) nb = 4096;
+        hipLaunchKernelGGL(zero_sets_kernel, dim3((unsigned)nb, 1, (unsigned)ctx->bn), dim3(256), 0, st, reinterpret_cast<double2*>(V), n2,
+                           ctx->bstride);
+        HIP_TRY(ctx, hipGetLastError());
+    } else HIP_TRY(ctx, hipMemsetAsync(V, 0, sizeof(double) * Np * Np, st));
+    return 0;
+}
+
 int trtri_lower(gpry_ctx* ctx, const double* L, double* V, double* T, int64_t Np) {
     hipStream_t st = ctx->stream;
+    ctx->kinv_from_row = 0;
+    if (factor_rows_apply(ctx, Np)) {
+        TrtriPlan* plr = nullptr;
+        GPRY_TRY(trtri_plan_get(ctx, Np, &plr));
+        GPRY_TRY(rows_clear_and_reserve(ctx, plr->rows, V, Np, st));
+        for (size_t i = 0; i < plr->rows.blocks.size(); i++) GPRY_TRY(rows_stage(ctx, plr->rows, L, V, T, Np, i, st));
+        return 0;
+    }
     const bool single_wave = Np <= 128;
     const bool clear_in_diag = !single_wave && Np <= 1024;
     const bool tp_min_clear = ctx->tp && !single_wave;
@@ -316,7 +473,9 @@
 struct TrtriPipe {
     const double* L = nullptr; double* V = nullptr; double* T = nullptr;
     int64_t Np = 0; TrtriPlan* pl = nullptr; size_t next = 0; bool active = false;
+    bool rows = false;
     hipStream_t side = nullptr;
+    hipStream_t kside = nullptr;
 };
 static TrtriPipe* pipe_of(gpry_ctx* ctx) {
     if (!ctx->trtri_pipe) ctx->trtri_pipe = new TrtriPipe();
@@ -344,6 +503,26 @@
     if (!ctx->stream2) return 1;
     TrtriPlan* pl = nullptr;
     GPRY_TRY(trtri_plan_get(ctx, Np, &pl));
+    ctx->kinv_from_row = 0;
+    if (factor_rows_apply(ctx, Np)) {
+        const size_t nb = pl->rows.blocks.size();
+        if (nb < 2) return 1;
+        if (!ctx->stream3) HIP_TRY(ctx, hipStreamCreateWithFlags(&ctx->stream3, hipStreamNonBlocking));
+        while (ctx->ev_pool.size() < 2 * nb + 3) {
+            hipEvent_t ev;
+            HIP_TRY(ctx, hipEventCreateWithFlags(&ev, hipEventDisableTiming));
+            ctx->ev_pool.push_back(ev);
+        }
+        pp->L = L; pp->V = V; pp->T = T; pp->Np = Np; pp->pl = pl; pp->next = 0; pp->rows = true;
+        pp->side = ctx->stream2; pp->kside = ctx->stream3;
+        hipEvent_t ev0 = ctx->ev_pool[nb];
+        HIP_TRY(ctx, hipEventRecord(ev0, ctx->stream));
+        HIP_TRY(ctx, hipStreamWaitEvent(pp->side, ev0, 0));
+        GPRY_TRY(rows_clear_and_reserve(ctx, pl->rows, V, Np, pp->side));
+        pp->active = true;
+        return 0;
+    }
+    pp->rows = false;
     if (pl->phases.size() < 2 || pl->leaf != 1) return 1;
     while (ctx->ev_pool.size() < pl->phases.size() + 2) {
         hipEvent_t ev;
@@ -377,6 +556,17 @@
     TrtriPipe* pp = static_cast<TrtriPipe*>(ctx->trtri_pipe);
     if (!pp || !pp->active) return 0;
     const TrtriPlan* pl = pp->pl;
+    if (pp->rows) {
+        const RowsPlan& rp = pl->rows;
+        if (pp->next + 1 >= rp.blocks.size() || rp.blocks[pp->next].r1 / 64 != blocks_done) return 0;
+        hipEvent_t ev = ctx->ev_pool[pp->next];
+        HIP_TRY(ctx, hipEventRecord(ev, ctx->stream));
+        HIP_TRY(ctx, hipStreamWaitEvent(pp->side, ev, 0));
+        GPRY_TRY(rows_stage(ctx, rp, pp->L, pp->V, pp->T, pp->Np, pp->next, pp->side, pp->kside,
+                            ctx->ev_pool[rp.blocks.size() + 2 + pp->next]));
+        pp->next++;
+        return 0;
+    }
     if (pp->next + 1 >= pl->phases.size() || pl->phases[pp->next].blocks_done != blocks_done) return 0;
     hipEvent_t ev = ctx->ev_pool[pp->next];
     HIP_TRY(ctx, hipEventRecord(ev, ctx->stream));
@@ -390,9 +580,17 @@
     if (!pp || !pp->active) return gpry_fail(ctx, -1, "trtri_pipeline_finish without begin");
     pp->active = false;
     const TrtriPlan* pl = pp->pl;
-    hipEvent_t evd = ctx->ev_pool[pl->phases.size() + 1];
+    hipEvent_t evd = ctx->ev_pool[(pp->rows ? pl->rows.blocks.size() : pl->phases.size()) + 1];
     HIP_TRY(ctx, hipEventRecord(evd, pp->side));
     HIP_TRY(ctx, hipStreamWaitEvent(ctx->stream, evd, 0));
+    if (pp->rows) {
+        hipEvent_t evk = ctx->ev_pool[2 * pl->rows.blocks.size() + 2];
+        HIP_TRY(ctx, hipEventRecord(evk, pp->kside));
+        HIP_TRY(ctx, hipStreamWaitEvent(ctx->stream, evk, 0));
+        for (; pp->next < pl->rows.blocks.size(); pp->next++)
+            GPRY_TRY(rows_stage(ctx, pl->rows, pp->L, pp->V, pp->T, pp->Np, pp->next, ctx->stream));
+        return 0;
+    }
     for (; pp->next < pl->phases.size(); pp->next++) GPRY_TRY(trtri_phase_run(ctx, pp, pp->next, ctx->stream));
     return 0;
 }
@@ -402,6 +600,7 @@
     if (!pp || !pp->active) return;
     pp->active = false;
     if (pp->side) (void)hipStreamSynchronize(pp->side);
+    if (pp->rows && pp->kside) (void)hipStreamSynchronize(pp->kside);
 }
 
 int lauum_lower(gpry_ctx* ctx, const double* V, double* Kinv, int64_t Np) {
@@ -434,7 +633,12 @@
     TrtriPlan* pl = nullptr;
     GPRY_TRY(trtri_plan_get(ctx, Np, &pl));
     int m = 1;
-    for (size_t lev = 0; lev < pl->count.size(); lev++) {
+    const bool rows = factor_rows_apply(ctx, Np);
+    if (rows) {
+        const int64_t need = (int64_t)pl->rows.max_slices * pl->rows.b * Np;
+        if (need > 0) m = std::max<int>(2, (int)((need + Np * Np - 1) / (Np * Np)));
+    }
+    for (size_t lev = 0; lev < pl->count.size() && !rows; lev++) {
         if (pl->seg_t[lev] > 0 && Np <= ctx->opt_gemm_streamk) {
             if (pl->sk_t[lev].max_slices > m) m = pl->sk_t[lev].max_slices;
             if (pl->sk_v[lev].max_slices > m) m = pl->sk_v[lev].max_slices;
@@ -443,7 +647,8 @@
             if (ns > m) m = ns;
         }
     }
-    if (Np >= 512 && Np <= ctx->opt_gemm_streamk) {
+    if (kinv_rows_apply(ctx, Np)) {
+    } else if (Np >= 512 && Np <= ctx->opt_gemm_streamk) {
         if (pl->sk_lauum.max_slices > m) m = pl->sk_lauum.max_slices;
     } else {
         const int nsplit = splitk_count((Np / 128) * (Np / 128 + 1) / 2, Np);
diff --git a/gpry_amd/csrc/common.h b/gpry_amd/csrc/common.h
--- a/gpry_amd/csrc/common.h
+++ b/gpry_amd/csrc/common.h
@@ -32,6 +32,7 @@
 struct gpry_ctx {
     int device = 0;
     hipStream_t stream = nullptr;
+    hipStream_t stream3 = nullptr;
     hipStream_t stream2 = nullptr;
     std::vector<hipEvent_t> ev_pool;
     char err[1024] = {0};
@@ -164,6 +165,11 @@
     int64_t opt_gemm_streamk = 5632;
     int64_t opt_topk_host = 16384;
     int opt_factor_pipeline = 1;
+    int64_t opt_trtri_rows = 1024;
+    int64_t opt_kinv_rows = 0;
+    int64_t opt_rows_min = 2304;
+    double* chain_kinv = nullptr;
+    int64_t kinv_from_row = 0;
     int opt_factor_pipeline_min = 1280;
     void* chol_plan = nullptr;
 
@@ -310,7 +316,8 @@
     KM_B_UPPER = 4,
     KM_AT_LOWER = 5
 };
-enum GemmEpi { EPI_STORE = 0, EPI_STORE_NEG = 1, EPI_SUB = 2, EPI_SUMSQ = 3 };
+enum GemmEpi { EPI_STORE = 0, EPI_STORE_NEG = 1, EPI_SUB = 2, EPI_SUMSQ = 3,
+               EPI_ACC = 4 };
 enum GemmTileMap { TM_ROWMAJOR = 0, TM_SWEEP = 1, TM_BALANCED = 2 };
 #define TM_SWEEP_SMALL (1 << 12)
 
@@ -334,6 +341,7 @@
     int small64;
     int bn, bz_div;
     int64_t bstride;
+    int kshift;
 };
 __device__ __forceinline__ void gemm_block_z(const GemmArgs& g, int z, int* tb, int* item) {
     if (g.bn > 1) { *tb = z / g.bz_div; *item = z - *tb * g.bz_div; }
@@ -420,6 +428,9 @@
 void trtri_pipeline_abort(gpry_ctx* ctx);
 void trtri_pipe_free(gpry_ctx* ctx);
 int lauum_lower(gpry_ctx* ctx, const double* V, double* Kinv, int64_t Np);
+bool factor_rows_apply(const gpry_ctx* ctx, int64_t Np);
+bool kinv_rows_apply(const gpry_ctx* ctx, int64_t Np);
+int kinv_rows_finish(gpry_ctx* ctx, const double* V, double* Kinv, int64_t Np);
 int factor_chain_slices(gpry_ctx* ctx, int64_t Np, int* slices);
 int solve_alpha(gpry_ctx* ctx, const double* V, const double* y, double* z, double* alpha,
                 int64_t Np);
diff --git a/gpry_amd/csrc/ctx.hip b/gpry_amd/csrc/ctx.hip
--- a/gpry_amd/csrc/ctx.hip
+++ b/gpry_amd/csrc/ctx.hip
@@ -231,6 +231,7 @@
     (void)hipSetDevice(ctx->device);
     (void)hipStreamSynchronize(ctx->stream);
     if (ctx->stream2) (void)hipStreamSynchronize(ctx->stream2);
+    if (ctx->stream3) (void)hipStreamSynchronize(ctx->stream3);
     timers_collect(ctx);
     serve_free(ctx);
     trtri_plan_free(ctx);
@@ -251,6 +252,7 @@
     if (ctx->hbres) (void)hipHostFree(ctx->hbres);
     (void)hipStreamDestroy(ctx->stream);
     if (ctx->stream2) (void)hipStreamDestroy(ctx->stream2);
+    if (ctx->stream3) (void)hipStreamDestroy(ctx->stream3);
     for (hipEvent_t ev : ctx->ev_pool) (void)hipEventDestroy(ev);
     for (hipStream_t st : ctx->tp_streams) (void)hipStreamDestroy(st);
     for (hipEvent_t ev : ctx->tp_events) (void)hipEventDestroy(ev);
@@ -283,6 +285,9 @@
     OPT_INT("chol_overlap", opt_chol_overlap, 0, 1, c->lml_cache = false),
     OPT_INT("factor_pipeline", opt_factor_pipeline, 0, 1, (void)0),
     OPT_INT("factor_pipeline_min", opt_factor_pipeline_min, 0, BIG, (void)0),
+    OPT_INT("trtri_rows", opt_trtri_rows, 0, 4096, c->opt_trtri_rows = round_up(c->opt_trtri_rows, 128); c->lml_cache = false),
+    OPT_INT("kinv_rows", opt_kinv_rows, 0, 4096, if (c->opt_kinv_rows > 1) c->opt_kinv_rows = round_up(c->opt_kinv_rows, 128); c->lml_cache = false),
+    OPT_INT("rows_min", opt_rows_min, 0, BIG, c->lml_cache = false),
     OPT_INT("gemm_dma", opt_gemm_dma, 0, 1, (void)0),
     OPT_INT("gemm_streamk", opt_gemm_streamk, 0, BIG, trtri_plan_free(c)),
     OPT_INT("gemm_small", opt_gemm_small, 0, BIG, c->lml_cache = false),
diff --git a/gpry_amd/csrc/gemm_dma.hip b/gpry_amd/csrc/gemm_dma.hip
--- a/gpry_amd/csrc/gemm_dma.hip
+++ b/gpry_amd/csrc/gemm_dma.hip
@@ -26,6 +26,9 @@
         case EPI_STORE: hipLaunchKernelGGL((gemm_dma_kernel<AT, BT, EPI_STORE>), grid, dim3(256), 0, st, g); break;
         case EPI_STORE_NEG: hipLaunchKernelGGL((gemm_dma_kernel<AT, BT, EPI_STORE_NEG>), grid, dim3(256), 0, st, g); break;
         case EPI_SUB: hipLaunchKernelGGL((gemm_dma_kernel<AT, BT, EPI_SUB>), grid, dim3(256), 0, st, g); break;
+        case EPI_ACC:
+            if constexpr (AT && !BT) { hipLaunchKernelGGL((gemm_dma_kernel<AT, BT, EPI_ACC>), grid, dim3(256), 0, st, g); break; }
+            return gpry_fail(ctx, -1, "gemm_dma: the accumulating epilogue is built for C += A^T B alone");
         default: return gpry_fail(ctx, -1, "gemm_dma: bad epilogue %d", epi);
     }
     HIP_TRY(ctx, hipGetLastError());
diff --git a/gpry_amd/csrc/gemm_dma_body.h b/gpry_amd/csrc/gemm_dma_body.h
--- a/gpry_amd/csrc/gemm_dma_body.h
+++ b/gpry_amd/csrc/gemm_dma_body.h
@@ -121,7 +121,7 @@
     int kbeg = 0, kend = K;
     if (g.kmode == KM_A_LOWER) kend = min(K, row0 + BM);
     else if (g.kmode == KM_B_LOWER) kbeg = min(K, col0);
-    else if (g.kmode == KM_AT_LOWER_B_LOWER) kbeg = min(K, max(row0, col0));
+    else if (g.kmode == KM_AT_LOWER_B_LOWER) kbeg = min(K, max(0, max(row0, col0) - g.kshift));
     else if (g.kmode == KM_B_UPPER) kend = min(K, col0 + BN);
     else if (g.kmode == KM_AT_LOWER) kbeg = min(K, row0);
     bool partial = g.nsplit > 1;
@@ -153,6 +153,13 @@
             for (int j = 0; j < 4; j++)
 #pragma unroll
                 for (int q = 0; q < 4; q++) acc[i][j][q] = -cbase[(int64_t)(i * 16 + 4 * q) * g.ldc + j * 16];
+    } else if (EPI == EPI_ACC && !partial && row0 < g.kshift) {
+#pragma unroll
+        for (int i = 0; i < 4; i++)
+#pragma unroll
+            for (int j = 0; j < 4; j++)
+#pragma unroll
+                for (int q = 0; q < 4; q++) acc[i][j][q] = cbase[(int64_t)(i * 16 + 4 * q) * g.ldc + j * 16];
     } else {
 #pragma unroll
         for (int i = 0; i < 4; i++)
@@ -260,7 +267,7 @@
             for (int q = 0; q < 4; q++) {
                 double* p = cbase + (int64_t)(mi * 16 + 4 * q) * g.ldc + ni * 16;
                 const double v = acc[mi][ni][q];
-                if (EPI == EPI_STORE || partial) *p = v;
+                if (EPI == EPI_STORE || EPI == EPI_ACC || partial) *p = v;
                 else *p = -v;
             }
 }
diff --git a/gpry_amd/gpr.py b/gpry_amd/gpr.py
--- a/gpry_amd/gpr.py
+++ b/gpry_amd/gpr.py
@@ -53,7 +53,7 @@
         return False
 
 
-_FIT_CONTEXT_OPTIONS = ("chol", "chol_overlap", "chol_stacked", "factor_pipeline", "factor_pipeline_min", "gemm_dma", "gemm_streamk",
+_FIT_CONTEXT_OPTIONS = ("chol", "chol_overlap", "chol_stacked", "factor_pipeline", "factor_pipeline_min", "trtri_rows", "kinv_rows", "rows_min", "gemm_dma", "gemm_streamk",
                         "gemm_small", "lml_small", "lml_cache", "lml_batch", "lml_batch_mb", "lml_schedule", "lml_streams",
                         "tp_block", "tp_tail")
 
diff --git a/include/gpry_hip.h b/include/gpry_hip.h
--- a/include/gpry_hip.h
+++ b/include/gpry_hip.h
@@ -242,6 +242,7 @@
 int gpry_timing_get(gpry_ctx* ctx, const char* name, double* total_ms, int64_t* count);
 int gpry_microbench(gpry_ctx* ctx, int kind, int64_t bytes, double* value);
 
+int gpry_debug_lml_scratch(gpry_ctx* ctx, int which, double* out);
 int gpry_debug_gemm(gpry_ctx* ctx, const double* A, const double* B, double* C, int M, int N,
                     int K, int a_trans, int b_trans, int epi, int kmode, int lower_only,
                     int tile_map);
```

After: 67.18 million. -1.3%, worse.
